# kangxiongbin/HyLight

Hardware: AMD Instinct MI355X
Metric: long-read all-vs-all overlaps/sec (higher is better)
Workload: dtype u8/int32

## Files before the change

### hylight_amd/csrc/ava.h

```cpp
#pragma once
#include <vector>

#include "common.h"
#include "paf_io.h"

namespace hlmi {

constexpr int CHAIN_PRED = 64;
constexpr int BLOCK_MIN = 32;
constexpr int BLOCK_MAX = 256;
constexpr int BAND_W = 64;
constexpr int BAND_PAD = 12;
constexpr int NARROW_W = 16;
constexpr int NARROW_PAD = 5;
constexpr int NARROW_DELTA = 5;
constexpr int EXT_MAX = 256;
constexpr int HALF_W = 32;
constexpr int HALF_DELTA = 7;
constexpr int ZDROP_STEP = 32;
constexpr int SHIFT_MAX = BAND_W - 2 * BAND_PAD - 1;
constexpr int MAX_MID_OCC = 1000000;
constexpr int NEG_INF = -(1 << 29);

inline int ext_rows(const hlmi_ava_opts &o) { return o.max_gap > EXT_MAX ? o.max_gap : EXT_MAX; }
inline int long_rows_cap(const hlmi_ava_opts &o) { return ext_rows(o) + BLOCK_MIN + SHIFT_MAX + BAND_W + 1; }

hlmi_ava_opts ava_opts_long();
hlmi_ava_opts ava_opts_short();

struct Mz {
    uint64_t x;
    uint64_t y;
};

struct DevReads {
    static constexpr size_t PAD = 64;
    size_t n = 0;
    uint64_t total = 0;
    DBuf<uint8_t> store;
    uint8_t *codes() const { return store.p + PAD; }
    void alloc_codes() {
        store.alloc(total + 2 * PAD);
        HIP_CHECK(hipMemsetAsync(store.p, 4, PAD, stream()));
        HIP_CHECK(hipMemsetAsync(store.p + PAD + total, 4, PAD, stream()));
    }
    DBuf<uint64_t> off;
    std::vector<uint64_t> h_off;
};
void upload_reads(const SeqSet &s, size_t lo, size_t hi, DevReads &out);
void upload_reads(const SeqSet &s, const std::vector<uint32_t> &ids, DevReads &out);
void subset_reads_device(const DevReads &all, const std::vector<uint32_t> &ids, DevReads &out);

struct DevSketch {
    size_t n = 0;
    DBuf<Mz> mz;
    DBuf<uint32_t> counts;
};
void sketch_device(const DevReads &r, int k, int w, int hpc, uint32_t rid_base, DevSketch &out);
int64_t sketch_device_into(const DevReads &r, int k, int w, int hpc, uint32_t rid_base, Mz *d_out, int64_t cap,
                           uint32_t *d_counts);

struct AvaInput {
    const DevReads *T = nullptr;
    const DevReads *Q = nullptr;
    const uint32_t *d_rank_t = nullptr;
    const uint32_t *d_rank_q = nullptr;
    uint64_t n_ranks = 0;
    const uint32_t *d_chunk_of_t = nullptr;
    uint32_t n_chunks = 1;
    const Mz *d_qmz = nullptr;
    std::vector<uint64_t> qmz_off;
    std::vector<uint32_t> t_query;
    uint64_t max_anchors = 0;
    uint64_t max_out_bytes = 0;
    int max_lanes = 0;
};
inline uint64_t ava_out_bytes(uint64_t rows, uint64_t ops) { return 4 * ops + 216 * rows; }

struct AvaRows {
    size_t n_rows = 0, n_ops = 0;
    DBuf<PafRec> recs;
    std::vector<DBuf<uint32_t>> ops_parts;
    std::vector<uint64_t> ops_part_len;
    const uint32_t *ops_base = nullptr;
    std::vector<uint64_t> chunk_row_start;
    uint64_t refused_anchors = 0;
    double refused_shrink = 1.0;
};
void ava_device(const AvaInput &in, const hlmi_ava_opts &o, AvaRows &out);

void ava_files(const char *target_fa, const char *query_fa, const hlmi_ava_opts &o, const char *out_paf);

void name_ranks(const std::vector<std::string> &a, const std::vector<std::string> &b, std::vector<uint32_t> &ra,
                std::vector<uint32_t> &rb, std::vector<std::string> &name_of_rank);

void format_ava_row(const PafRec &r, const uint32_t *ops, const std::string &qname, const std::string &tname,
                    std::string &out);

}
```

### hylight_amd/csrc/ava_align.hip

```cpp
#include <algorithm>
#include <memory>
#include <type_traits>

#include "ava_internal.h"
#include "dev_prims.h"
#include "wave_ops.h"

namespace hlmi {

namespace {
constexpr int WG = 256;
constexpr int WAVES = WG / 64;
constexpr int SEQ_T_MAX = EXT_MAX + BAND_W;
constexpr int NR_SHORT = 128;
constexpr int WIDE_SHORT = 128;
inline dim3 grid1(size_t n) { return dim3(cdiv(n ? n : 1, WG)); }

struct Task {
    uint32_t piece;
    uint16_t kind;
    uint16_t narrow;
    uint64_t qa, ta;
    int16_t m, n;
    int16_t dlo;
    int16_t trim;
};
constexpr uint16_t TASK_REV = 4;
constexpr uint16_t TASK_ONE = 8;
struct TaskOut {
    int32_t score;
    int32_t bi, bj;
    uint32_t runs_off, n_runs;
    uint32_t pad;
};
__device__ __forceinline__ uint32_t end_codes(uint32_t first_run, uint32_t last_run) { return (first_run & 15u) | (last_run & 15u) << 4; }

__global__ void piece_task_count_kernel(const Piece *pieces, size_t n, uint32_t *cnt) {
    size_t i = blockIdx.x * (size_t)blockDim.x + threadIdx.x;
    if (i < n) cnt[i] = pieces[i].n_fp + 1;
}

struct TaskRef { uint32_t pk, fp; };
struct PieceGeom {
    uint64_t qo, to;
    uint32_t ql, tl;
    uint32_t strand;
    uint32_t stub_cand;
};
struct TaskGeom {
    const TaskRef *ref;
    const PieceGeom *pg;
    const FixPt *fps;
};
__device__ __forceinline__ Task build_task(const PieceGeom &p, uint32_t piece, uint32_t kind, FixPt f0, FixPt f1, int ext_max) {
    const int ql = (int)p.ql, tl = (int)p.tl;
    const uint64_t qo = p.qo, to = p.to;
    const uint16_t rev = p.strand ? TASK_REV : 0;
    auto qaddr = [&](int pos) { return p.strand ? qo + (uint64_t)(ql - 1 - pos) : qo + (uint64_t)pos; };
    if (kind == 1) {
        const int qs = (int)f0.q, ts = (int)f0.t;
        const int m = qs < ext_max ? qs : ext_max, n2 = ts < m + BAND_W ? ts : m + BAND_W;
        return Task{piece, (uint16_t)(1u | rev), (uint16_t)(qs <= ext_max ? (qs + 1) << 1 : 0), qaddr(qs - 1),
                    to + (uint64_t)(ts - 1), (int16_t)m, (int16_t)n2, (int16_t)(-(BAND_W / 2 - 1)), 0};
    }
    if (kind == 2) {
        const int qe = (int)f0.q, te = (int)f0.t;
        const int m = ql - qe < ext_max ? ql - qe : ext_max, n2 = tl - te < m + BAND_W ? tl - te : m + BAND_W;
        return Task{piece, (uint16_t)(2u | rev), (uint16_t)(ql - qe <= ext_max ? (ql - qe + 1) << 1 : 0), qaddr(qe),
                    to + (uint64_t)te, (int16_t)m, (int16_t)n2, (int16_t)(-(BAND_W / 2 - 1)), 0};
    }
    const int q0 = (int)f0.q, t0 = (int)f0.t, m = (int)f1.q - q0, n2 = (int)f1.t - t0;
    const int delta = n2 - m, ad = delta < 0 ? -delta : delta;
    const bool lng = m > BLOCK_MAX || n2 > BLOCK_MAX;
    const bool narrow = !lng && ad <= NARROW_DELTA;
    const int lw = ad <= HALF_DELTA ? HALF_W : BAND_W;
    return Task{piece, rev, (uint16_t)(narrow ? 1 : 0), qaddr(q0), to + (uint64_t)t0, (int16_t)m, (int16_t)n2,
                (int16_t)((delta < 0 ? delta : 0) - (narrow ? NARROW_PAD : lng ? (lw - 1 - ad) / 2 : BAND_PAD)), 0};
}
__global__ __launch_bounds__(WG) void task_ref_kernel(const Piece *pieces, const uint32_t *task_off, size_t n, const uint32_t *qlen,
                                                       const uint32_t *tlen, const uint64_t *qoff, const uint64_t *toff,
                                                       const FixPt *fps, int stub_oh, int ext_max, TaskRef *task_ref, PieceGeom *pg) {
    const int lane = threadIdx.x & 63;
    const size_t wave = (blockIdx.x * (size_t)blockDim.x + threadIdx.x) >> 6;
    const size_t n_waves = ((size_t)gridDim.x * blockDim.x) >> 6;
    for (size_t i = wave; i < n; i += n_waves) {
        const Piece p = pieces[i];
        const uint32_t n_tasks = p.n_fp + 1;
        TaskRef *out = task_ref + task_off[i];
        for (uint32_t k = (uint32_t)lane; k < n_tasks; k += 64) {
            const uint32_t kind = k == 0 ? 1u : (k == p.n_fp ? 2u : 0u);
            out[k] = TaskRef{(uint32_t)i | kind << 30, p.fp_off + (k == 0 ? 0u : k - 1)};
        }
        if (lane == 0) {
            const uint32_t ql = qlen[p.q], tl = tlen[p.t];
            uint32_t cand = 0;
            if (stub_oh >= 0) {
                const FixPt a = fps[p.fp_off], b = fps[p.fp_off + p.n_fp - 1];
                const uint32_t dq = (uint32_t)(ext_max + stub_oh), dt = (uint32_t)(ext_max + BAND_W + stub_oh);
                cand = ((a.q > dq && a.t > dt) || (ql - b.q > dq && tl - b.t > dt)) ? 1u : 0u;
            }
            pg[i] = PieceGeom{qoff[p.q], toff[p.t], ql, tl, p.strand, cand};
        }
    }
}

__global__ __launch_bounds__(WG) void task_ref_lane_kernel(const Piece *pieces, const uint32_t *task_off, size_t n, const uint32_t *qlen,
                                                            const uint32_t *tlen, const uint64_t *qoff, const uint64_t *toff,
                                                            const FixPt *fps, int stub_oh, int ext_max, TaskRef *task_ref, PieceGeom *pg) {
    const size_t i = blockIdx.x * (size_t)blockDim.x + threadIdx.x;
    if (i >= n) return;
    const Piece p = pieces[i];
    const uint32_t n_tasks = p.n_fp + 1;
    TaskRef *out = task_ref + task_off[i];
    for (uint32_t k = 0; k < n_tasks; ++k) {
        const uint32_t kind = k == 0 ? 1u : (k == p.n_fp ? 2u : 0u);
        out[k] = TaskRef{(uint32_t)i | kind << 30, p.fp_off + (k == 0 ? 0u : k - 1)};
    }
    const uint32_t ql = qlen[p.q], tl = tlen[p.t];
    uint32_t cand = 0;
    if (stub_oh >= 0) {
        const FixPt a = fps[p.fp_off], b = fps[p.fp_off + p.n_fp - 1];
        const uint32_t dq = (uint32_t)(ext_max + stub_oh), dt = (uint32_t)(ext_max + BAND_W + stub_oh);
        cand = ((a.q > dq && a.t > dt) || (ql - b.q > dq && tl - b.t > dt)) ? 1u : 0u;
    }
    pg[i] = PieceGeom{qoff[p.q], toff[p.t], ql, tl, p.strand, cand};
}

struct AlignArgs {
    Task *tasks;
    TaskGeom geom;
    size_t n_tasks;
    const uint32_t *list;
    size_t n_list;
    const uint8_t *qcodes, *tcodes;
    long long q_total, t_total;
    int match, mismatch, go, ge, ambi;
    int go2, ge2;
    int end_bonus;
    int ext_max;
    int ext_all_long;
    int ungapped;
    int kmax;
    int kgap1;
    int kgap2;
    int one_ok;
    int kext_plain;
    int kext_bonus;
    int trim_ok;
    int kshift;
    TaskOut *out;
    uint32_t *runs;
    uint32_t cap_runs;
    uint32_t *counters;
    uint32_t run_buf_cap;
    uint8_t *cls_bare;
    uint8_t *defer_flag;
    const uint32_t *defer_list, *defer_count;
};

__device__ __forceinline__ uint32_t wave_excl_sum_u32(uint32_t v, int lane, uint32_t &total) {
    (void)lane;
    const uint32_t x = wave_prefix_sum_incl_dpp(v);
    total = (uint32_t)__builtin_amdgcn_readlane((int)x, 63);
    return x - v;
}

constexpr uint32_t RUN_CHUNK = 4096;
constexpr uint32_t RUN_CHUNK_SMALL = 256;
__device__ __forceinline__ uint32_t pool_take(const AlignArgs &a, uint32_t n, uint32_t &chunk_off, uint32_t &chunk_left,
                                              bool &ok, uint32_t chunk = RUN_CHUNK) {
    if (n > chunk_left) {
        const uint32_t want = n > chunk ? n : chunk;
        chunk_off = atomicAdd(&a.counters[0], want);
        chunk_left = want;
        if ((unsigned long long)chunk_off + want > a.cap_runs) { a.counters[1] = 1; chunk_left = 0; ok = false; return 0; }
    }
    const uint32_t off = chunk_off;
    chunk_off += n;
    chunk_left -= n;
    return off;
}

__device__ __forceinline__ uint32_t load_codes4(const uint8_t *base, long long idx, long long total) {
    if (idx >= 0 && idx + 4 <= total) {
        uint32_t v;
        __builtin_memcpy(&v, base + idx, 4);
        return v;
    }
    uint32_t v = 0;
    for (int k = 0; k < 4; ++k) v |= (uint32_t)(idx + k >= 0 && idx + k < total ? base[idx + k] : 4) << (8 * k);
    return v;
}
__device__ __forceinline__ uint32_t comp_codes4(uint32_t x) {
    const uint32_t n = x & 0x04040404u;
    return (x ^ 0x03030303u) & ~((n >> 1) | (n >> 2));
}
__device__ __forceinline__ uint32_t load_window4(const uint8_t *codes, long long total, long long a0, bool down, bool comp, int x) {
    uint32_t v = down ? __builtin_bswap32(load_codes4(codes, a0 - x - 3, total)) : load_codes4(codes, a0 + x, total);
    if (comp) v = comp_codes4(v);
    return v;
}

__device__ __forceinline__ uint32_t load_window4p(const uint8_t *codes, long long a0, bool down, bool comp, int x) {
    uint32_t v;
    __builtin_memcpy(&v, codes + (down ? a0 - x - 3 : a0 + x), 4);
    if (down) v = __builtin_bswap32(v);
    if (comp) v = comp_codes4(v);
    return v;
}


enum { ST_BASES = 0, ST_BASES_SQUARE, ST_BASES_NARROW, ST_BASES_WIDE, ST_FAST, ST_DP, ST_DP_ROWS, ST_NARROW_SMALL, ST_WIDE_ONE, ST_STUB_EXT, ST_EXT_CERT, ST_EXT_DP_ROW, ST_EXT_DP_K, ST_LONG, ST_BASES_LONG, N_ALIGN_STATS };
constexpr int NR_SMALL = 64;
constexpr uint8_t CLS_LONG = 5;
constexpr uint8_t CLS_LONG32 = 7;
constexpr uint8_t CLS_UNGAPPED = 6;

__device__ __forceinline__ uint64_t load_codes8(const uint8_t *base, long long idx, long long total) {
    if (idx >= 0 && idx + 8 <= total) {
        uint64_t v;
        __builtin_memcpy(&v, base + idx, 8);
        return v;
    }
    uint64_t v = 0;
    for (int k = 0; k < 8; ++k) v |= (uint64_t)(idx + k >= 0 && idx + k < total ? base[idx + k] : 4) << (8 * k);
    return v;
}
__device__ __forceinline__ uint64_t load_window8(const uint8_t *codes, long long total, long long a0, bool down, bool comp, int x) {
    uint64_t v = down ? __builtin_bswap64(load_codes8(codes, a0 - x - 7, total)) : load_codes8(codes, a0 + x, total);
    if (comp) {
        const uint64_t n = v & 0x0404040404040404ull;
        v = (v ^ 0x0303030303030303ull) & ~((n >> 1) | (n >> 2));
    }
    return v;
}

__device__ __forceinline__ uint64_t load_window8p(const uint8_t *codes, long long a0, bool down, bool comp, int x) {
    uint64_t v;
    __builtin_memcpy(&v, codes + (down ? a0 - x - 7 : a0 + x), 8);
    if (down) v = __builtin_bswap64(v);
    if (comp) {
        const uint64_t n = v & 0x0404040404040404ull;
        v = (v ^ 0x0303030303030303ull) & ~((n >> 1) | (n >> 2));
    }
    return v;
}

template <int PASS>
__global__ __launch_bounds__(WG) __attribute__((amdgpu_waves_per_eu(PASS == 1 ? 4 : 5))) void classify_kernel(AlignArgs a, uint8_t *cls, unsigned long long *stats) {
    __shared__ unsigned long long s_stat[WAVES][N_ALIGN_STATS];
    constexpr int CMP_PIECES = PASS == 1 ? 64 * (BLOCK_MAX / 8) : 1;
    __shared__ uint8_t s_mm[WAVES][CMP_PIECES], s_up[WAVES][CMP_PIECES], s_dn[WAVES][CMP_PIECES];
    __shared__ uint64_t s_qa[WAVES][PASS == 1 ? 64 : 1], s_ta[WAVES][PASS == 1 ? 64 : 1];
    __shared__ uint32_t s_geo[WAVES][PASS == 1 ? 64 : 1], s_amb[WAVES][2];
    const int lane = threadIdx.x & 63;
    const size_t tid = blockIdx.x * (size_t)blockDim.x + threadIdx.x;
    const size_t n_thr = (size_t)gridDim.x * blockDim.x;
    uint32_t chunk_off = 0, chunk_left = 0;
    uint32_t st[N_ALIGN_STATS] = {0, 0, 0, 0, 0, 0, 0, 0, 0, 0, 0, 0, 0, 0, 0};
    const size_t n_units = PASS == 1 ? a.n_tasks : (size_t)*a.defer_count;
    const size_t rounds = (n_units + n_thr - 1) / n_thr;
    TaskRef ref_n{0, 0};
    uint32_t ti_n = 0;
    if (PASS == 1) { if (tid < n_units) ref_n = a.geom.ref[tid]; }
    else if (tid < n_units) ti_n = a.defer_list[tid];
    for (size_t r = 0; r < rounds; ++r) {
        const size_t u = r * n_thr + tid;
        bool live = u < n_units;
        const size_t ti = PASS == 1 || !live ? u : (size_t)ti_n;
        TaskRef ref = ref_n;
        if (PASS == 2 && live) ref = a.geom.ref[ti];
        {
            const size_t un = u + n_thr;
            if (PASS == 1) { if (un < n_units) ref_n = a.geom.ref[un]; }
            else if (un < n_units) ti_n = a.defer_list[un];
        }
        Task tk{};
        bool held = false;
        bool bare = false;
        if (live) {
            const uint32_t pc = ref.pk & 0x3fffffffu, kind = ref.pk >> 30;
            const PieceGeom pg = a.geom.pg[pc];
            held = PASS == 1 && kind != 0 && pg.stub_cand != 0;
            bare = a.cls_bare != nullptr && pg.stub_cand != 0;
            const FixPt f0 = a.geom.fps[ref.fp];
            FixPt f1{0, 0};
            if (kind == 0) f1 = a.geom.fps[ref.fp + 1];
            tk = build_task(pg, pc, kind, f0, f1, a.ext_max);
        }
        const int m = tk.m, n = tk.n;
        uint8_t c = 2;
        bool try_fast = false;
        if (live) {
            if (m <= 0 || n <= 0 || held) c = 0;
            else if ((tk.kind & 3) == 0) {
                if (m > BLOCK_MAX || n > BLOCK_MAX)
                    c = (n > m ? n - m : m - n) <= HALF_DELTA ? CLS_LONG32 : CLS_LONG;
                else { c = tk.narrow ? (m <= NR_SHORT ? 1 : 3) : 2; try_fast = (m == n); }
            } else if ((m < n - tk.dlo ? m : n - tk.dlo) > EXT_MAX) { c = CLS_LONG32; tk.dlo = (int16_t)(-(HALF_W / 2 - 1)); }
            else if (a.ext_all_long) c = CLS_LONG;
            if (c == 2 && (m < n - tk.dlo ? m : n - tk.dlo) <= WIDE_SHORT) c = 4;
        }
        if (PASS == 1 && live) {
            const bool defer = c != 0 && a.kmax >= 0 && ((tk.kind & 3) != 0 || (m != n && c != CLS_LONG && c != CLS_LONG32));
            a.defer_flag[ti] = defer ? 1 : 0;
            if (defer) { live = false; try_fast = false; }
        }
        int k = 0, mpos[3] = {0, 0, 0}, last_x = -1;
        bool ambig = false, shift_ok = false;
        if constexpr (PASS == 1) {
            const int wv = threadIdx.x >> 6;
            uint8_t *own = s_mm[wv], *mm = s_mm[wv], *mup = s_up[wv], *mdn = s_dn[wv];
            const uint32_t nch = try_fast ? (uint32_t)(m + 7) >> 3 : 0u;
            const uint32_t incl = wave_prefix_sum_incl_dpp(nch), tot = (uint32_t)__builtin_amdgcn_readlane((int)incl, 63);
            const uint32_t st0 = incl - nch;
            for (uint32_t c = (uint32_t)lane; c < tot; c += 64) own[c] = 0;
            if (lane < 2) s_amb[wv][lane] = 0;
            s_qa[wv][lane] = tk.qa; s_ta[wv][lane] = tk.ta;
            s_geo[wv][lane] = st0 | (uint32_t)m << 16 | ((tk.kind & TASK_REV) ? 0x80000000u : 0u);
            __builtin_amdgcn_s_waitcnt(0xc07f);
            __builtin_amdgcn_wave_barrier();
            if (nch) own[st0] = (uint8_t)lane;
            __builtin_amdgcn_s_waitcnt(0xc07f);
            __builtin_amdgcn_wave_barrier();
            int carry = 0;
            constexpr int CU = 4;
            for (uint32_t c0 = 0; c0 < tot; c0 += 64 * CU) {
                int ow[CU], xs[CU], left[CU];
                bool rv[CU];
#pragma unroll
                for (int u = 0; u < CU; ++u) {
                    const uint32_t c = c0 + 64u * u + (uint32_t)lane;
                    int o = c < tot ? (int)own[c] : 0;
                    o = wave_prefix_max_incl_dpp(o);
                    o = o > carry ? o : carry;
                    carry = __builtin_amdgcn_readlane(o, 63);
                    const uint32_t geo = s_geo[wv][o];
                    ow[u] = o;
                    xs[u] = (int)(c - (geo & 0xffffu)) * 8;
                    left[u] = c < tot ? (int)(geo >> 16 & 0x7fffu) - xs[u] : 0;
                    rv[u] = (geo >> 31) != 0;
                }
                uint64_t q8[CU], t8[CU];
                uint32_t q_end = 0, t_end = 0;
#pragma unroll
                for (int u = 0; u < CU; ++u) {
                    q8[u] = t8[u] = 0;
                    if (left[u] > 0) {
                        q8[u] = load_window8p(a.qcodes, (long long)s_qa[wv][ow[u]], rv[u], rv[u], xs[u]);
                        t8[u] = load_window8p(a.tcodes, (long long)s_ta[wv][ow[u]], false, false, xs[u]);
                        if (u == CU - 1 && lane == 63 && a.kshift) {
                            q_end = (uint32_t)load_window8p(a.qcodes, (long long)s_qa[wv][ow[u]], rv[u], rv[u], xs[u] + 8) & 0xffu;
                            t_end = (uint32_t)load_window8p(a.tcodes, (long long)s_ta[wv][ow[u]], false, false, xs[u] + 8) & 0xffu;
                        }
                    }
                }
                int nq[CU], nt[CU];
                if (a.kshift) {
#pragma unroll
                    for (int u = 0; u < CU; ++u) {
                        const int q_after = u + 1 < CU ? __builtin_amdgcn_readlane((int)((uint32_t)q8[u + 1 < CU ? u + 1 : u] & 0xffu), 0) : (int)q_end;
                        const int t_after = u + 1 < CU ? __builtin_amdgcn_readlane((int)((uint32_t)t8[u + 1 < CU ? u + 1 : u] & 0xffu), 0) : (int)t_end;
                        nq[u] = wave_shl1((int)((uint32_t)q8[u] & 0xffu), q_after);
                        nt[u] = wave_shl1((int)((uint32_t)t8[u] & 0xffu), t_after);
                    }
                }
#pragma unroll
                for (int u = 0; u < CU; ++u) {
                    if (left[u] <= 0) continue;
                    const uint64_t keep = left[u] >= 8 ? ~0ull : (1ull << (8 * left[u])) - 1ull;
                    uint64_t d = (q8[u] ^ t8[u]) & keep;
                    if ((q8[u] | t8[u]) & keep & 0x0404040404040404ull) atomicOr(&s_amb[wv][ow[u] >> 5], 1u << (ow[u] & 31));
                    d = (d | d >> 1 | d >> 2) & 0x0101010101010101ull;
                    auto squeeze = [](uint64_t f) {
                        return (uint8_t)((((uint32_t)f * 0x10204080u) >> 28) | (((uint32_t)(f >> 32) * 0x10204080u) >> 28) << 4);
                    };
                    mm[c0 + 64u * u + (uint32_t)lane] = squeeze(d);
                    if (a.kshift) {
                        const uint64_t q9 = q8[u] >> 8 | (uint64_t)(uint32_t)nq[u] << 56, t9 = t8[u] >> 8 | (uint64_t)(uint32_t)nt[u] << 56;
                        uint64_t du = q9 ^ t8[u], dd = q8[u] ^ t9;
                        du = (du | du >> 1 | du >> 2) & 0x0101010101010101ull;
                        dd = (dd | dd >> 1 | dd >> 2) & 0x0101010101010101ull;
                        mup[c0 + 64u * u + (uint32_t)lane] = squeeze(du);
                        mdn[c0 + 64u * u + (uint32_t)lane] = squeeze(dd);
                    }
                }
            }
            __builtin_amdgcn_s_waitcnt(0xc07f);
            __builtin_amdgcn_wave_barrier();
            if (try_fast) {
                ambig = (s_amb[wv][lane >> 5] >> (lane & 31)) & 1u;
                for (uint32_t j = 0; j < nch && k <= a.kmax + a.kshift; ++j) {
                    uint32_t bits = mm[st0 + j];
                    while (bits) {
                        const int y = __ffs((int)bits) - 1;
                        bits &= bits - 1;
                        if (k < 3) mpos[k] = (int)(8 * j) + y;
                        ++k;
                    }
                }
            }
            if (try_fast && !ambig && a.kshift && k == a.kmax + 1) {
                const int p1 = mpos[0], pk = mpos[k - 1];
                uint32_t any_up = 0, any_dn = 0;
                for (int j = p1 >> 3; j <= (pk - 1) >> 3; ++j) {
                    uint32_t keepb = 0xffu;
                    if (j == p1 >> 3) keepb &= 0xffu << (p1 & 7);
                    if (j == (pk - 1) >> 3) keepb &= 0xffu >> (7 - ((pk - 1) & 7));
                    any_up |= mup[st0 + (uint32_t)j] & keepb;
                    any_dn |= mdn[st0 + (uint32_t)j] & keepb;
                }
                shift_ok = any_up != 0 && any_dn != 0;
            }
            if (try_fast && k > 0 && !ambig) {
                for (int j = (int)nch - 1; j >= 0; --j) {
                    const uint32_t bits = mm[st0 + (uint32_t)j];
                    if (bits) { last_x = 8 * j + 31 - __clz((int)bits); break; }
                }
            }
            __builtin_amdgcn_wave_barrier();
        }
        bool fast = try_fast && !ambig && k <= a.kmax;
        if (shift_ok) fast = true;
        uint32_t runs[7];
        uint32_t nr = 0;
        int fast_score = a.match * (m - k) - a.mismatch * k;
        uint32_t ext_flag = 0;
        int ext_take = -1;
        if (PASS == 2 && live && c != 0 && (tk.kind & 3) != 0 && a.kmax >= 0) {
            const bool rev = (tk.kind & TASK_REV) != 0, left = (tk.kind & 3) == 1;
            const int L = m < n ? m : n;
            const int end_row = (int)(tk.narrow >> 1) - 1;
            const bool bonus_row = a.end_bonus != 0 && end_row >= 0 && end_row <= n + (BAND_W / 2 - 1);
            bool same = !bonus_row || L == end_row;
            int allow = -1, k_ext = 0;
            bool amb_ext = false;
            if (a.go2 > 0 && a.ge > a.ge2 && a.end_bonus == 0 && a.one_ok) {
                int g = (a.go2 - a.go + (a.ge - a.ge2) - 1) / (a.ge - a.ge2);
                g = g < 1 ? 1 : g;
                allow = (a.go2 + a.ge2 * g - 1) / (a.match + a.mismatch);
            }
            const int k_want = bonus_row ? (L == end_row ? a.kext_bonus : 0) : a.kext_plain;
            int x1 = -1, x2 = -1;
            auto more = [&]() { return same || (!amb_ext && (k_ext <= allow || k_ext <= k_want)); };
            auto take8 = [&](int x, uint64_t q8, uint64_t t8) {
                const int rest = L - x;
                const uint64_t keep = rest >= 8 ? ~0ull : (1ull << (8 * rest)) - 1ull;
                uint64_t d = (q8 ^ t8) & keep;
                amb_ext |= ((q8 | t8) & keep & 0x0404040404040404ull) != 0;
                d = (d | d >> 1 | d >> 2) & 0x0101010101010101ull;
                if (d && x2 < 0) {
                    const int y1 = (__ffsll((long long)d) - 1) >> 3;
                    if (x1 < 0) { x1 = x + y1; const uint64_t d2 = d & (d - 1); if (d2) x2 = x + ((__ffsll((long long)d2) - 1) >> 3); }
                    else x2 = x + y1;
                }
                k_ext += __popcll(d);
                same = same && d == 0 && !amb_ext;
            };
            for (int x = 0; x < L && more(); x += 16) {
                const uint64_t q8 = load_window8p(a.qcodes, (long long)tk.qa, left != rev, rev, x);
                const uint64_t t8 = load_window8p(a.tcodes, (long long)tk.ta, left, false, x);
                uint64_t q8b = 0, t8b = 0;
                if (x + 8 < L) {
                    q8b = load_window8p(a.qcodes, (long long)tk.qa, left != rev, rev, x + 8);
                    t8b = load_window8p(a.tcodes, (long long)tk.ta, left, false, x + 8);
                }
                take8(x, q8, t8);
                if (x + 8 < L && more()) take8(x + 8, q8b, t8b);
            }
            if (!same && !amb_ext && k_ext <= allow) { tk.kind |= TASK_ONE; ++st[ST_WIDE_ONE]; }
            if (same) {
                runs[nr++] = (uint32_t)L << 4 | OP_EQ;
                fast_score = a.match * L;
                ext_flag = L == end_row ? 0x80000000u : 0u;
                fast = true;
                c = 0;
            } else if (!amb_ext && k_ext >= 1 && k_ext <= k_want) {
                int take = L;
                if (!bonus_row && a.match * x1 >= a.match * (L - 1) - a.mismatch) take = x1;
                const int subs = take == L ? k_ext : 0;
                int prev = 0;
                if (take > 0) {
                    if (subs >= 1) {
                        if (x1 > 0) runs[nr++] = (uint32_t)x1 << 4 | OP_EQ;
                        if (subs == 2 && x2 == x1 + 1) { runs[nr++] = 2u << 4 | OP_X; prev = x2 + 1; }
                        else {
                            runs[nr++] = 1u << 4 | OP_X; prev = x1 + 1;
                            if (subs == 2) {
                                runs[nr++] = (uint32_t)(x2 - prev) << 4 | OP_EQ;
                                runs[nr++] = 1u << 4 | OP_X; prev = x2 + 1;
                            }
                        }
                    }
                    if (take > prev) runs[nr++] = (uint32_t)(take - prev) << 4 | OP_EQ;
                }
                if (left) for (uint32_t i = 0; i < nr / 2; ++i) { const uint32_t v = runs[i]; runs[i] = runs[nr - 1 - i]; runs[nr - 1 - i] = v; }
                fast_score = a.match * (take - subs) - a.mismatch * subs;
                ext_flag = bonus_row && take == end_row ? 0x80000000u : 0u;
                ext_take = take;
                fast = true;
                c = 0;
                ++st[ST_EXT_CERT];
            } else if (bonus_row && L != end_row) ++st[ST_EXT_DP_ROW];
            else ++st[ST_EXT_DP_K];
        } else if (PASS == 2 && live && c != 0 && (tk.kind & 3) == 0 && m != n && a.kmax >= 0) {
            const bool rev = (tk.kind & TASK_REV) != 0;
            const int mn = m < n ? m : n, gap = n > m ? n - m : m - n;
            const bool del = n > m;
            const int want = a.kgap1 && gap == 1 ? (a.kgap2 ? 3 : 2) : 1;
            int found_a = 0, found_b = 0, a1 = mn, a2 = mn, a3 = mn, b1 = -1, b2 = -1, b3 = -1;
            bool amb = false;
            const int sq = m > n ? m - n : 0, st_ = n > m ? n - m : 0;
            for (int x = 0; x < mn && (found_a < want || found_b < want); x += 8) {
                const bool da = found_a < want, db = found_b < want;
                const int e0 = mn - 8 - x;
                uint64_t q8 = 0, t8 = 0, q8e = 0, t8e = 0;
                if (da) { q8 = load_window8p(a.qcodes, (long long)tk.qa, rev, rev, x); t8 = load_window8p(a.tcodes, (long long)tk.ta, false, false, x); }
                if (db) { q8e = load_window8p(a.qcodes, (long long)tk.qa, rev, rev, e0 + sq); t8e = load_window8p(a.tcodes, (long long)tk.ta, false, false, e0 + st_); }
                const int left = mn - x;
                if (da) {
                    const uint64_t keep = left >= 8 ? ~0ull : (1ull << (8 * left)) - 1ull;
                    amb |= ((q8 | t8) & keep & 0x0404040404040404ull) != 0;
                    uint64_t d = (q8 ^ t8) & keep;
                    d = (d | d >> 1 | d >> 2) & 0x0101010101010101ull;
                    while (d && found_a < want) {
                        const int y = (__ffsll((long long)d) - 1) >> 3;
                        d &= d - 1;
                        if (found_a == 0) a1 = x + y; else if (found_a == 1) a2 = x + y; else a3 = x + y;
                        ++found_a;
                    }
                }
                if (db) {
                    const uint64_t keep = left >= 8 ? ~0ull : ~0ull << (8 * (8 - left));
                    amb |= ((q8e | t8e) & keep & 0x0404040404040404ull) != 0;
                    uint64_t d = (q8e ^ t8e) & keep;
                    d = (d | d >> 1 | d >> 2) & 0x0101010101010101ull;
                    while (d && found_b < want) {
                        const int z = 7 - (__clzll((long long)d) >> 3);
                        d &= ~(0xffull << (8 * z));
                        if (found_b == 0) b1 = e0 + z; else if (found_b == 1) b2 = e0 + z; else b3 = e0 + z;
                        ++found_b;
                    }
                }
            }
            int p_star = -1, xpos = -1, xpos2 = -1;
            if (!amb) {
                if (b1 < a1) p_star = b1 + 1;
                else if (want >= 2 && b2 < a1) { p_star = b2 + 1; xpos = b1; }
                else if (want >= 2 && b1 < a2) { p_star = b1 + 1; xpos = a1; }
            }
            if (p_star < 0 && !amb && want == 3) {
                int ps = -1, x1 = -1, x2 = -1;
                const int mab = a1 < b2 ? a1 : b2, Mab = a1 > b2 ? a1 : b2, m2 = a2 < b1 ? a2 : b1, M2 = a2 > b1 ? a2 : b1;
                if (b2 >= 0 && b3 < mab) { ps = b3 + 1; x1 = b2; x2 = b1; }
                else if (a1 < mn && b1 >= 0 && Mab < m2) { ps = Mab + 1; x1 = a1; x2 = b1; }
                else if (a2 < mn && M2 < a3) { ps = M2 + 1; x1 = a1; x2 = a2; }
                if (ps >= 0 && a1 < b1) {
                    auto load_s = [&](int x) { return del ? load_window8p(a.qcodes, (long long)tk.qa, rev, rev, x) : load_window8p(a.tcodes, (long long)tk.ta, false, false, x); };
                    auto load_l = [&](int x) { return del ? load_window8p(a.tcodes, (long long)tk.ta, false, false, x) : load_window8p(a.qcodes, (long long)tk.qa, rev, rev, x); };
                    bool far_ne = false, near_ne = false, ambx = false;
                    for (int x = a1; x < b1 && !far_ne; x += 8) {
                        const uint64_t s8 = load_s(x), l8 = load_l(x + 2);
                        const int left = b1 - x;
                        const uint64_t keep = left >= 8 ? ~0ull : (1ull << (8 * left)) - 1ull;
                        ambx |= ((s8 | l8) & keep & 0x0404040404040404ull) != 0;
                        far_ne = ((s8 ^ l8) & keep) != 0;
                    }
                    for (int x = a1 + 1; x <= b1 && !near_ne; x += 8) {
                        const uint64_t s8 = load_s(x), l8 = load_l(x - 1);
                        const int left = b1 + 1 - x;
                        const uint64_t keep = left >= 8 ? ~0ull : (1ull << (8 * left)) - 1ull;
                        ambx |= ((s8 | l8) & keep & 0x0404040404040404ull) != 0;
                        near_ne = ((s8 ^ l8) & keep) != 0;
                    }
                    if (far_ne && near_ne && !ambx) { p_star = ps; xpos = x1; xpos2 = x2; }
                }
            }
            if (p_star < 0 && !amb && b1 >= 0) last_x = b1;
            if (p_star >= 0) {
                auto seg = [&](int from, int to) {
                    int prev = from;
                    for (int k = 0; k < 2; ++k) {
                        const int xp = k ? xpos2 : xpos;
                        if (xp < from || xp >= to) continue;
                        if (xp > prev) runs[nr++] = (uint32_t)(xp - prev) << 4 | OP_EQ;
                        if (nr && xp == prev && prev > from && (runs[nr - 1] & 15u) == OP_X) runs[nr - 1] += 1u << 4;
                        else runs[nr++] = 1u << 4 | OP_X;
                        prev = xp + 1;
                    }
                    if (to > prev) runs[nr++] = (uint32_t)(to - prev) << 4 | OP_EQ;
                };
                seg(0, p_star);
                runs[nr++] = (uint32_t)gap << 4 | (del ? OP_D : OP_I);
                seg(p_star, mn);
                const int subs = (xpos >= 0 ? 1 : 0) + (xpos2 >= 0 ? 1 : 0);
                int gap_cost = a.go + a.ge * gap;
                if (a.go2 && a.go2 + a.ge2 * gap < gap_cost) gap_cost = a.go2 + a.ge2 * gap;
                fast_score = a.match * (mn - subs) - a.mismatch * subs - gap_cost;
                fast = true;
                c = 0;
            }
        } else if (fast) {
            c = 0;
            int prev = 0, xs = -1, xe = -1;
            for (int i = 0; i < k; ++i) {
                const int x = mpos[i];
                if (x == xe) { xe = x + 1; continue; }
                if (xs >= 0) { runs[nr++] = (uint32_t)(xe - xs) << 4 | OP_X; prev = xe; }
                if (x > prev) runs[nr++] = (uint32_t)(x - prev) << 4 | OP_EQ;
                xs = x; xe = x + 1;
            }
            if (xs >= 0) { runs[nr++] = (uint32_t)(xe - xs) << 4 | OP_X; prev = xe; }
            if (m > prev) runs[nr++] = (uint32_t)(m - prev) << 4 | OP_EQ;
        }
        if (bare) nr = 0;
        uint32_t wave_total;
        const uint32_t mine = wave_excl_sum_u32(nr, lane, wave_total);
        uint32_t base = 0;
        bool ok = true;
        if (wave_total) {
            if (lane == 0) base = pool_take(a, wave_total, chunk_off, chunk_left, ok);
            base = (uint32_t)__shfl((int)base, 0, 64);
            ok = __shfl((int)ok, 0, 64) != 0;
        }
        if (fast) {
            if (ok) for (uint32_t q = 0; q < nr; ++q) a.runs[base + mine + q] = runs[q];
            const bool ext = (tk.kind & 3) != 0;
            const int L = ext_take >= 0 ? ext_take : (m < n ? m : n);
            a.out[ti] = TaskOut{fast_score, ext ? L : m, ext ? L : n, base + mine, ok ? nr : 0, (nr ? end_codes(runs[0], runs[nr - 1]) : 0u) | ext_flag};
        } else if (live && c == 0) {
            a.out[ti] = TaskOut{0, 0, 0, 0, 0, 0};
        }
        int m_dp = m;
        if (live && !fast && (c == 1 || c == 3) && a.kmax >= 0 && last_x >= 0 && a.trim_ok && !a.ungapped) {
            const int mn = m < n ? m : n;
            int T = mn - 1 - last_x;
            T = T < mn - 1 ? T : mn - 1;
            if (T > 0) {
                tk.m = (int16_t)(m - T); tk.n = (int16_t)(n - T); tk.trim = (int16_t)T;
                m_dp = m - T;
                c = m_dp <= NR_SHORT ? 1 : 3;
            }
        }
        if (live) {
            if (a.ungapped && c != 0) c = CLS_UNGAPPED;
            cls[ti] = bare ? 0 : c;
            if (a.cls_bare) a.cls_bare[ti] = bare ? c : 0;
            if (c != 0) a.tasks[ti] = tk;
            if (held) ++st[ST_STUB_EXT];
            else if (m > 0 && n > 0) {
                const uint32_t bases = (uint32_t)(m + n);
                st[ST_BASES] += bases;
                if ((tk.kind & 3) == 0 && m == n) st[ST_BASES_SQUARE] += bases;
                if (c == 0) ++st[ST_FAST];
                else {
                    ++st[ST_DP];
                    if (c == CLS_LONG || c == CLS_LONG32) { ++st[ST_LONG]; st[ST_BASES_LONG] += bases; st[ST_DP_ROWS] += (uint32_t)(m < n - tk.dlo ? m : n - tk.dlo); }
                    else if (c == 2 || c == 4) { st[ST_BASES_WIDE] += bases; st[ST_DP_ROWS] += (uint32_t)(m < n - tk.dlo ? m : n - tk.dlo); }
                    else { st[ST_BASES_NARROW] += bases; st[ST_DP_ROWS] += (uint32_t)m_dp; if (c == 1 && m_dp < NR_SMALL && !bare) ++st[ST_NARROW_SMALL]; }
                }
            }
        }
    }
#pragma unroll
    for (int k = 0; k < N_ALIGN_STATS; ++k) {
        unsigned long long v = st[k];
#pragma unroll
        for (int o = 32; o > 0; o >>= 1) v += __shfl_xor(v, o, 64);
        if (lane == 0) s_stat[threadIdx.x >> 6][k] = v;
    }
    __syncthreads();
    if (threadIdx.x < N_ALIGN_STATS) {
        unsigned long long v = 0;
        for (int w = 0; w < WAVES; ++w) v += s_stat[w][threadIdx.x];
        if (v) atomicAdd(&stats[threadIdx.x], v);
    }
}

__global__ void task_rows_key_kernel(const Task *tasks, const uint32_t *list, size_t n, uint32_t *key) {
    size_t i = blockIdx.x * (size_t)blockDim.x + threadIdx.x;
    if (i < n) key[i] = (uint32_t)tasks[list[i]].m >> 2;
}


__global__ void task_rows_desc_key_kernel(const Task *tasks, const uint32_t *list, size_t n, uint32_t *key) {
    size_t i = blockIdx.x * (size_t)blockDim.x + threadIdx.x;
    if (i >= n) return;
    const Task &t = tasks[list[i]];
    const int rows = (int)t.m < (int)t.n - (int)t.dlo ? (int)t.m : (int)t.n - (int)t.dlo;
    key[i] = 0xffffu - (uint32_t)(rows < 0 ? 0 : rows);
}

constexpr int DP_BIAS = 1 << 24;
constexpr int NT_PAD = 16;
constexpr int NT_EXTRA = NT_PAD + NARROW_DELTA + NARROW_W + 7;
enum { PL_DIAG = 0, PL_EGEF, PL_EEXT, PL_FEXT, PL_NE, N_PLANES };

__device__ __forceinline__ uint32_t shift_in(uint32_t acc, bool bit) {
#if defined(__HIP_DEVICE_COMPILE__)
    const unsigned long long m = __ballot(bit);
    unsigned long long co;
    asm("v_addc_co_u32 %0, %1, %2, %2, %3" : "=v"(acc), "=s"(co) : "v"(acc), "s"(m));
#endif
    return acc;
}

struct NarrowWalk {
    const uint32_t *pl;
    int chunks;
    int lb;
    int m, n, dlo;
    int wmask;
    bool keep_order;
    int trim;
    __device__ __forceinline__ uint32_t word(int plane, int c, int lane) const { return pl[(plane * chunks + c) * 64 + lane]; }
};
struct WalkScore {
    int match, mismatch, go, ge;
    int total;
};
__device__ uint32_t narrow_walk(const NarrowWalk &w, uint32_t *out, uint32_t total, uint32_t *buf = nullptr, uint32_t cap = 0,
                                WalkScore *ws = nullptr, uint32_t *ends = nullptr) {
    int i = w.m, j = w.n, state = 0;
    uint32_t cur_op = OP_EQ, cur_len = (uint32_t)w.trim, n_runs = 0, e_first = 0, e_last = 0;
    auto put = [&]() {
        if (!n_runs) e_first = cur_op;
        e_last = cur_op;
        if (out) out[w.keep_order ? n_runs : total - 1 - n_runs] = cur_len << 4 | cur_op;
        else if (n_runs < cap) buf[n_runs] = cur_len << 4 | cur_op;
        ++n_runs;
        if (ws) ws->total += cur_op == OP_EQ ? ws->match * (int)cur_len
                           : (cur_op == OP_X ? -ws->mismatch * (int)cur_len : -(ws->go + ws->ge * (int)cur_len));
    };
    for (int it = 0; (i > 0 || j > 0) && it < 4 * (EXT_MAX + SEQ_T_MAX); ++it) {
        uint32_t op, len;
        if (i == 0) {
            op = OP_D; len = (uint32_t)j; j = 0;
        } else {
            const int d = w.lb + ((j - i - w.dlo) & w.wmask);
            const int c = (i - 1) >> 5, sh = 31 - ((i - 1) & 31);
            const uint32_t dg = w.word(PL_DIAG, c, d) >> sh;
            const uint32_t ne = w.word(PL_NE, c, d) >> sh;
            const uint32_t eg = w.word(PL_EGEF, c, d) >> sh;
            const uint32_t ee = w.word(PL_EEXT, c, (d - 1) & 63) >> sh;
            const int i2 = i > 1 ? i - 2 : 0;
            const uint32_t fe = w.word(PL_FEXT, i2 >> 5, (d + 1) & 63) >> (31 - (i2 & 31));
            const int st = state != 0 ? state : ((dg & 1u) ? 0 : ((eg & 1u) ? 1 : 2));
            if (st == 0) {
                const uint32_t inv = ~dg;
                const int r = inv ? __ffs((int)inv) - 1 : 32;
                const bool isx = (ne & 1u) != 0;
                const uint32_t flip = isx ? ~ne : ne;
                int l = flip ? __ffs((int)flip) - 1 : 32;
                l = l < r ? l : r;
                op = isx ? OP_X : OP_EQ; len = (uint32_t)l;
                i -= l; j -= l;
                state = 0;
            } else if (st == 1) {
                op = OP_D; len = 1;
                state = (ee & 1u) ? 1 : 0;
                --j;
            } else {
                op = OP_I; len = 1;
                state = (i > 1 && (fe & 1u)) ? 2 : 0;
                --i;
            }
        }
        if (op == cur_op) cur_len += len;
        else { if (cur_len) put(); cur_op = op; cur_len = len; }
    }
    if (cur_len) put();
    if (ends) *ends = w.keep_order ? end_codes(e_first, e_last) : end_codes(e_last, e_first);
    return n_runs;
}
constexpr int RUN_BUF_NARROW = 48, RUN_BUF_WIDE = 128;

template <bool AMBI, int NR_CHUNKS>
__device__ __forceinline__ void narrow_rows(const AlignArgs &a, int rows, int m, int dlo, int l, const uint8_t *sq,
                                            const uint8_t *st, uint32_t (*pl)[NR_CHUNKS][64], int lane, int &Hend) {
    const int go = a.go, ge = a.ge, goe = go + ge, gel = ge * l, goel = go + ge * l;
    const int j0 = dlo + l;
    int H = j0 == 0 ? DP_BIAS : (j0 > 0 ? DP_BIAS - (go + ge * j0) : 0);
    int G = H - goe;
    uint32_t a0 = 0, a1 = 0, a2 = 0, a3 = 0, a4 = 0;
    const uint8_t *tp = st + NT_PAD + dlo + l - 1;
    int v_match = a.match, v_mis = -a.mismatch;
    asm volatile("" : "+v"(v_match), "+v"(v_mis));
    auto row = [&](int i, int qa, int t2) {
        const bool ne = qa != t2;
        int s = ne ? v_mis : v_match;
        if (AMBI) s = (qa | t2) > 3 ? -a.ambi : s;
        const int mm = H + s;
        const int f = row_shl1_z(G);
        const int ht = mm > f ? mm : f;
        const int e = row_shr1(row_prefix_max_incl_dpp(ht + gel), 0) - goel;
        const int h = ht > e ? ht : e;
        const int fo = h - goe, fe = f - ge;
        a0 = shift_in(a0, mm == h);
        a1 = shift_in(a1, e >= f);
        a2 = shift_in(a2, e + go > h);
        a3 = shift_in(a3, fe > fo);
        a4 = shift_in(a4, ne);
        G = fo > fe ? fo : fe;
        H = h;
        if (i == m) Hend = h;
    };
    int qa = sq[0], t2 = tp[1];
    int i = 1;
    for (; i < rows; i += 2) {
        const int qb = sq[i], tb = tp[i + 1], qc = sq[i + 1], tc = tp[i + 2];
        row(i, qa, t2);
        row(i + 1, qb, tb);
        qa = qc; t2 = tc;
        if (((i + 1) & 31) == 0) {
            const int c = ((i + 1) >> 5) - 1;
            pl[PL_DIAG][c][lane] = a0; pl[PL_EGEF][c][lane] = a1; pl[PL_EEXT][c][lane] = a2; pl[PL_FEXT][c][lane] = a3;
            pl[PL_NE][c][lane] = a4;
        }
    }
    if (i == rows) row(i, qa, t2);
    if (rows & 31) {
        const int c = rows >> 5, up = 32 - (rows & 31);
        pl[PL_DIAG][c][lane] = a0 << up; pl[PL_EGEF][c][lane] = a1 << up; pl[PL_EEXT][c][lane] = a2 << up;
        pl[PL_FEXT][c][lane] = a3 << up; pl[PL_NE][c][lane] = a4 << up;
    }
}

template <int NR_MAX>
__global__ __launch_bounds__(WG) void align_narrow_kernel(AlignArgs a) {
    constexpr int NR_CHUNKS = NR_MAX / 32, NQ_STEPS = NR_MAX / 64, NT_STEPS = NR_MAX / 64 + 1;
    __shared__ uint32_t s_pl[WAVES][N_PLANES][NR_CHUNKS][64];
    __shared__ __attribute__((aligned(4))) uint8_t s_q[WAVES * 4][NR_MAX + 4];
    __shared__ __attribute__((aligned(4))) uint8_t s_t[WAVES * 4][NR_MAX + NT_EXTRA];
    __shared__ uint32_t s_runs[WAVES * 4][RUN_BUF_NARROW];
    const int lane = threadIdx.x & 63, g = lane >> 4, l = lane & 15, wv = threadIdx.x >> 6;
    const size_t wave = (blockIdx.x * (size_t)blockDim.x + threadIdx.x) >> 6;
    const size_t n_waves = ((size_t)gridDim.x * blockDim.x) >> 6;
    uint32_t (*pl)[NR_CHUNKS][64] = s_pl[wv];
    uint8_t *sq = s_q[wv * 4 + g], *st = s_t[wv * 4 + g];
    uint32_t chunk_off = 0, chunk_left = 0;
    const size_t n_quads = (a.n_list + 3) / 4;
    for (size_t qd = wave; qd < n_quads; qd += n_waves) {
        const size_t li = qd * 4 + g;
        const bool live = li < a.n_list;
        size_t ti = 0;
        Task tk{};
        if (live) { ti = a.list[li]; tk = a.tasks[ti]; }
        const int m = tk.m, n = tk.n, dlo = tk.dlo;
        bool ambig = false;
        if (live) {
            const bool rev = (tk.kind & TASK_REV) != 0;
            uint32_t vq[NQ_STEPS], vt[NT_STEPS];
#pragma unroll
            for (int r = 0; r < NQ_STEPS; ++r) {
                const int x = 4 * (l + 16 * r);
                vq[r] = 0;
                if (x < m) vq[r] = load_window4p(a.qcodes, (long long)tk.qa, rev, rev, x);
            }
#pragma unroll
            for (int r = 0; r < NT_STEPS; ++r) {
                const int x = 4 * (l + 16 * r);
                vt[r] = 0;
                if (x < n) vt[r] = load_window4p(a.tcodes, (long long)tk.ta, false, false, x);
            }
#pragma unroll
            for (int r = 0; r < NQ_STEPS; ++r) {
                const int x = 4 * (l + 16 * r);
                if (x < m) { *(uint32_t *)(sq + x) = vq[r]; ambig |= (vq[r] & 0x04040404u) != 0; }
            }
#pragma unroll
            for (int r = 0; r < NT_STEPS; ++r) {
                const int x = 4 * (l + 16 * r);
                if (x < n) { *(uint32_t *)(st + NT_PAD + x) = vt[r]; ambig |= (vt[r] & 0x04040404u) != 0; }
            }
        }
        __builtin_amdgcn_s_waitcnt(0);
        __builtin_amdgcn_wave_barrier();
// ... 1232 lines not shown

template <bool WRITE>
__global__ __launch_bounds__(WG) void assemble_lane_kernel(AsmArgs a, uint32_t *n_ops, uint8_t *valid, const uint64_t *ops_off,
                                                            uint32_t *ops, PafRec *recs, uint64_t *ord_hi, uint64_t *ord_lo) {
    const size_t idx = blockIdx.x * (size_t)blockDim.x + threadIdx.x;
    if (idx >= a.n_pieces) return;
    const size_t i = !WRITE && a.plist ? (size_t)a.plist[idx] : idx;
    if (WRITE && !valid[i]) return;
    const Piece p = a.pieces[i];
    const FixPt *fp = a.fps + p.fp_off;
    const TaskOut *to = a.tout + a.task_off[i];
    const uint32_t n_tasks = p.n_fp + 1;
    const bool bare = a.bare && a.pg[i].stub_cand != 0;
    uint32_t *w = WRITE ? ops + ops_off[i] : nullptr;
    long long score = 0;
    unsigned long long nmatch = 0, blen = 0;
    uint32_t slots = 0;
    uint32_t pend = 0;
    uint32_t carry_code = 99;
    int li = 0, lj = 0, ri = 0, rj = 0;
    for (uint32_t t = 0; t < n_tasks; ++t) {
        const TaskOut r = to[t];
        bool keep = true;
        if (t == 0 || t == n_tasks - 1)
            keep = !(r.score + ((r.pad & 0x80000000u) ? a.end_bonus : 0) <= 0 || (r.n_runs == 0 && !bare));
        if (!keep) continue;
        if (t == 0) { li = r.bi; lj = r.bj; }
        else if (t == n_tasks - 1) { ri = r.bi; rj = r.bj; }
        score += r.score;
        const uint32_t nr = bare ? 0u : r.n_runs;
        if (!nr) continue;
        const uint32_t first = r.pad & 15u, last = (r.pad >> 4) & 15u;
        const bool mrg = first == carry_code;
        carry_code = last;
        if (!WRITE) {
            slots += nr - (mrg ? 1u : 0u);
            continue;
        }
        for (uint32_t x = 0; x < nr; ++x) {
            const uint32_t run = a.runs[r.runs_off + x];
            blen += run >> 4;
            if ((run & 15u) == OP_EQ) nmatch += run >> 4;
            if (x == 0 && mrg) pend += (run >> 4) << 4;
            else {
                if (pend) w[slots++] = pend;
                pend = run;
            }
        }
    }
    if (!WRITE) {
        const bool ok = (slots > 0 || bare) && score >= a.min_dp_score;
        valid[i] = ok ? 1 : 0;
        n_ops[i] = ok ? slots : 0;
        if (a.late) a.late[i] = a.pg[i].stub_cand && !((slots > 0 || bare) && score >= a.stub_score) ? 1 : 0;
        return;
    }
    if (pend) w[slots++] = pend;
    const int qs = (int)fp[0].q - li, ts = (int)fp[0].t - lj;
    const int qe = (int)fp[p.n_fp - 1].q + ri, te = (int)fp[p.n_fp - 1].t + rj;
    const uint32_t ql = a.qlen[p.q];
    PafRec r{};
    r.qid = a.rank_q[p.q]; r.tid = a.rank_t[p.t];
    r.qlen = ql; r.tlen = a.tlen[p.t];
    r.qs = p.strand ? ql - (uint32_t)qe : (uint32_t)qs;
    r.qe = p.strand ? ql - (uint32_t)qs : (uint32_t)qe;
    r.ts = (uint32_t)ts; r.te = (uint32_t)te;
    r.nmatch = (uint32_t)nmatch; r.blen = (uint32_t)blen;
    r.flags = p.strand ? PF_REV : 0;
    r.chunk = a.chunk_of_t[p.t];
    r.cig_off = ops_off[i]; r.cig_n = slots; r.tie = 0;
    recs[i] = r;
    ord_hi[i] = (uint64_t)r.chunk << 32 | p.q;
    ord_lo[i] = (uint64_t)p.t << 43 | (uint64_t)p.strand << 42 | (uint64_t)(p.chain & 0x3fffffu) << 20 | (p.piece & 0xfffffu);
}

__global__ void late_tasks_kernel(const uint32_t *plist, size_t n, const Piece *pieces, const uint32_t *task_off, uint32_t *tasks,
                                  uint32_t *count) {
    size_t j = blockIdx.x * (size_t)blockDim.x + threadIdx.x;
    if (j == 0) *count = (uint32_t)(2 * n);
    if (j >= n) return;
    const uint32_t i = plist[j];
    tasks[2 * j] = task_off[i];
    tasks[2 * j + 1] = task_off[i] + pieces[i].n_fp;
}

__global__ __launch_bounds__(WG) void class_bases_kernel(const uint8_t *cls, const uint8_t *cls_bare, const Task *tasks, size_t n,
                                                          unsigned long long *out) {
    __shared__ unsigned long long s_sum[14];
    if (threadIdx.x < 14) s_sum[threadIdx.x] = 0;
    __syncthreads();
    for (size_t i = blockIdx.x * (size_t)blockDim.x + threadIdx.x; i < n; i += (size_t)gridDim.x * blockDim.x) {
        const int c = cls[i], cb = cls_bare ? cls_bare[i] : 0;
        if (!c && !cb) continue;
        const Task &t = tasks[i];
        int slot;
        if (c) slot = c == 1 ? ((int)t.m < NR_SMALL ? 0 : 1) : c == 3 ? 2 : c == 2 ? 3 : c == 4 ? 4 : c == CLS_LONG ? 5 : c == CLS_LONG32 ? 12 : 11;
        else slot = cb == 1 ? 6 : cb == 3 ? 7 : cb == 2 ? 8 : cb == 4 ? 9 : cb == CLS_LONG ? 10 : cb == CLS_LONG32 ? 13 : 11;
        atomicAdd(&s_sum[slot], (unsigned long long)((int)t.m + (int)t.n));
    }
    __syncthreads();
    if (threadIdx.x < 14 && s_sum[threadIdx.x]) atomicAdd(&out[threadIdx.x], s_sum[threadIdx.x]);
}

__global__ __launch_bounds__(WG) void list_ext_kernel(const Task *tasks, const uint32_t *list, size_t n, unsigned long long *out) {
    unsigned long long c = 0, r = 0;
    for (size_t i = blockIdx.x * (size_t)blockDim.x + threadIdx.x; i < n; i += (size_t)gridDim.x * blockDim.x) {
        const Task &t = tasks[list[i]];
        if (t.kind & 3) { ++c; r += (unsigned long long)(int)t.m; }
    }
#pragma unroll
    for (int o = 32; o > 0; o >>= 1) { c += __shfl_xor(c, o, 64); r += __shfl_xor(r, o, 64); }
    if ((threadIdx.x & 63) == 0 && c) { atomicAdd(out, c); atomicAdd(out + 1, r); }
}

__global__ void class_flag_kernel(const uint8_t *cls, size_t n, uint8_t v, uint8_t *flag) {
    size_t i = blockIdx.x * (size_t)blockDim.x + threadIdx.x;
    if (i < n) flag[i] = cls[i] == v ? 1 : 0;
}

__global__ void compact_rows_kernel(const uint32_t *idx, size_t n, const PafRec *recs, const uint64_t *hi,
                                    const uint64_t *lo, PafRec *orecs, uint64_t *ohi, uint64_t *olo) {
    size_t i = blockIdx.x * (size_t)blockDim.x + threadIdx.x;
    if (i >= n) return;
    orecs[i] = recs[idx[i]];
    ohi[i] = hi[idx[i]];
    olo[i] = lo[idx[i]];
}

__global__ __launch_bounds__(WG) void piece_long_flag_kernel(const Piece *pieces, size_t n, const FixPt *fps, const uint32_t *qlen,
                                                              const uint32_t *tlen, int ext_max, uint8_t *flag) {
    const int lane = threadIdx.x & 63;
    const size_t wave = (blockIdx.x * (size_t)blockDim.x + threadIdx.x) >> 6;
    const size_t n_waves = ((size_t)gridDim.x * blockDim.x) >> 6;
    for (size_t i = wave; i < n; i += n_waves) {
        const Piece p = pieces[i];
        const FixPt *fp = fps + p.fp_off;
        bool lng = false;
        if (lane == 0) {
            const FixPt a = fp[0], b = fp[p.n_fp - 1];
            const int ql = (int)qlen[p.q], tl = (int)tlen[p.t];
            auto rows = [&](int aq, int at) {
                const int m = aq < ext_max ? aq : ext_max, nn = at < m + BAND_W ? at : m + BAND_W;
                return m < nn + (BAND_W / 2 - 1) ? m : nn + (BAND_W / 2 - 1);
            };
            lng = rows((int)a.q, (int)a.t) > EXT_MAX || rows(ql - (int)b.q, tl - (int)b.t) > EXT_MAX;
        }
        for (uint32_t k = (uint32_t)lane; k + 1 < p.n_fp && !__any(lng); k += 64) {
            const FixPt f0 = fp[k], f1 = fp[k + 1];
            lng = lng || (int)(f1.q - f0.q) > BLOCK_MAX || (int)(f1.t - f0.t) > BLOCK_MAX;
        }
        const bool any = __any(lng);
        if (lane == 0) flag[i] = any ? 1 : 0;
    }
}
__global__ __launch_bounds__(WG) void piece_long_flag_lane_kernel(const Piece *pieces, size_t n, const FixPt *fps, const uint32_t *qlen,
                                                                   const uint32_t *tlen, int ext_max, uint8_t *flag) {
    const size_t i = blockIdx.x * (size_t)blockDim.x + threadIdx.x;
    if (i >= n) return;
    const Piece p = pieces[i];
    const FixPt *fp = fps + p.fp_off;
    FixPt f0 = fp[0];
    const FixPt b = fp[p.n_fp - 1];
    const int ql = (int)qlen[p.q], tl = (int)tlen[p.t];
    auto rows = [&](int aq, int at) {
        const int m = aq < ext_max ? aq : ext_max, nn = at < m + BAND_W ? at : m + BAND_W;
        return m < nn + (BAND_W / 2 - 1) ? m : nn + (BAND_W / 2 - 1);
    };
    bool lng = rows((int)f0.q, (int)f0.t) > EXT_MAX || rows(ql - (int)b.q, tl - (int)b.t) > EXT_MAX;
    for (uint32_t k = 1; k < p.n_fp && !lng; ++k) {
        const FixPt f1 = fp[k];
        lng = (int)(f1.q - f0.q) > BLOCK_MAX || (int)(f1.t - f0.t) > BLOCK_MAX;
        f0 = f1;
    }
    flag[i] = lng ? 1 : 0;
}
__global__ void gather_pieces_kernel(const Piece *src, const uint32_t *idx, size_t n, Piece *dst, uint32_t *n_fp) {
    size_t i = blockIdx.x * (size_t)blockDim.x + threadIdx.x;
    if (i >= n) return;
    const Piece p = src[idx[i]];
    dst[i] = p;
    if (n_fp) n_fp[i] = p.n_fp;
}
__global__ __launch_bounds__(WG) void move_fixed_points_kernel(Piece *pieces, size_t n, const uint32_t *off, uint32_t fp_base, const FixPt *src,
                                                                FixPt *dst) {
    const int lane = threadIdx.x & 63;
    const size_t wave = (blockIdx.x * (size_t)blockDim.x + threadIdx.x) >> 6;
    const size_t n_waves = ((size_t)gridDim.x * blockDim.x) >> 6;
    for (size_t i = wave; i < n; i += n_waves) {
        const Piece p = pieces[i];
        const uint32_t to = off[i];
        for (uint32_t k = (uint32_t)lane; k < p.n_fp; k += 64) dst[to + k] = src[p.fp_off + k];
        if (lane == 0) pieces[i].fp_off = fp_base + to;
    }
}
}

struct PieceSpan { struct { const Piece *p; } pieces; size_t n_pieces, n_fp; struct { const FixPt *p; } fps; };
static void align_span(const AvaInput &in, const hlmi_ava_opts &o, const uint32_t *d_qlen, const uint32_t *d_tlen,
                       const PieceSpan &ch, AlignOut &out) {
    out = AlignOut();
    const size_t P = ch.n_pieces;
    if (!P) return;
    DBuf<uint32_t> tcnt(P), toff(P);
    hipLaunchKernelGGL(piece_task_count_kernel, grid1(P), dim3(WG), 0, stream(), ch.pieces.p, P, tcnt.p);
    exclusive_scan_u32(tcnt.p, toff.p, P);
    const size_t NT = ch.n_fp + P;
    DBuf<Task> tasks(NT);
    if (P >= (1u << 30)) fail(HLMI_EINVAL, "more than 2^30 alignment pieces in one batch");
    DBuf<TaskRef> task_ref(NT);
    DBuf<PieceGeom> pgeom(P);
    if (NT <= 17 * P)
        hipLaunchKernelGGL(task_ref_lane_kernel, grid1(P), dim3(WG), 0, stream(), ch.pieces.p, toff.p, P, d_qlen, d_tlen, in.Q->off.p, in.T->off.p,
                           ch.fps.p, o.stub_oh, ext_rows(o), task_ref.p, pgeom.p);
    else
    hipLaunchKernelGGL(task_ref_kernel, dim3((unsigned)std::min<size_t>(cdiv(P, (size_t)WAVES), 256 * 32)), dim3(WG), 0, stream(),
                       ch.pieces.p, toff.p, P, d_qlen, d_tlen, in.Q->off.p, in.T->off.p, ch.fps.p, o.stub_oh, ext_rows(o), task_ref.p, pgeom.p);
    HIP_CHECK(hipGetLastError());
    DBuf<TaskOut> tout(NT);
    DBuf<uint32_t> counters(2);
    DBuf<unsigned long long> astats(N_ALIGN_STATS);
    constexpr size_t MAX_BLOCKS = 256 * 16;
    const size_t open_chunks = MAX_BLOCKS * (4 * WAVES * RUN_CHUNK + 2 * 4 * WAVES * RUN_CHUNK_SMALL) +
                               (size_t)3 * 256 * 32 * 8 * PK_WAVES * RUN_CHUNK_SMALL;
    size_t run_share = std::max<size_t>(NT * 12, 1 << 16);
    DBuf<uint32_t> runs;
    AsmArgs as{};
    as.pieces = ch.pieces.p; as.fps = ch.fps.p; as.task_off = toff.p; as.tout = tout.p; as.n_pieces = P;
    as.min_dp_score = o.min_dp_score; as.end_bonus = o.end_bonus;
    as.qlen = d_qlen; as.tlen = d_tlen; as.rank_q = in.d_rank_q; as.rank_t = in.d_rank_t; as.chunk_of_t = in.d_chunk_of_t;
    as.pg = pgeom.p; as.stub_score = o.min_dp_score + std::max(0, o.end_bonus);
    as.stage_cap = (uint32_t)ASM_STAGE;
    if (const char *e = hook("HLMI_ASM_STAGE_CAP")) as.stage_cap = (uint32_t)std::min(ASM_STAGE, std::max(0, atoi(e)));
    DBuf<uint32_t> nops(P);
    DBuf<uint8_t> valid(P), late(o.stub_oh >= 0 ? P : 0);
    DBuf<uint32_t> late_idx(o.stub_oh >= 0 ? P : 0);
    size_t n_late = 0;
    const unsigned nba = (unsigned)std::min<size_t>(cdiv(P, (size_t)WAVES), 256 * 32);
    const bool small_pieces = NT <= 17 * P && !hook("HLMI_ASM_WAVE");
    const int worst = std::max(std::max(o.match, o.mismatch), std::max(o.ambi, o.gap_open + o.gap_ext));
    const bool packed = worst > 0 && (long long)worst * (BLOCK_MAX + NARROW_W + 2) <= 4000 && o.match >= 0 && o.mismatch >= 0 &&
                        o.ambi >= 0 && o.gap_open >= 0 && o.gap_ext >= 0 && !hook("HLMI_NARROW_UNPACKED");
    const bool bare = o.stub_oh >= 0 && packed && !hook("HLMI_STUB_FULL_ROWS");
    as.bare = bare ? 1 : 0;
    if (long_rows_cap(o) > 32000) fail(HLMI_EINVAL, "max_gap %d: alignment tasks are limited to 32 000 rows", o.max_gap);
    bool ext_all_long = false;
    if (o.zdrop > 0) {
        const int D = std::max(std::max(o.mismatch, o.ambi), o.gap_open + o.gap_ext);
        const int rows_down = D > 0 ? (o.zdrop + D - 1) / D : EXT_MAX;
        ext_all_long = (long long)o.match * (EXT_MAX - rows_down) + std::max(o.end_bonus, 0) > o.zdrop;
    }
    const uint32_t long_chunks_cap = (uint32_t)(long_rows_cap(o) + 31) / 32, long_runs_cap = (uint32_t)(2 * long_rows_cap(o) + 64);
    constexpr unsigned LONG_BLOCKS_MAX = 256 * 8;
    struct LongLaunch { DBuf<uint32_t> list, planes, runs, ctl; };
    std::vector<std::unique_ptr<LongLaunch>> long_launches;
    struct LongReady { AlignArgs al; LongArgs la; unsigned nb; bool half, tb; const char *timer; };
    std::vector<LongReady> long_ready;
    hipEvent_t long_done = nullptr;
    bool long_pending = false, long_on_side = false;
    struct SideGuard {
        ~SideGuard() { if (hipStream_t s = side_stream_if_created()) (void)hipStreamSynchronize(s); }
    } side_guard;
    auto join_long = [&]() {
        if (!long_pending) return;
        if (long_on_side) {
            if (!long_done) HIP_CHECK(hipEventCreateWithFlags(&long_done, hipEventDisableTiming));
            HIP_CHECK(hipEventRecord(long_done, side_stream()));
            HIP_CHECK(hipStreamWaitEvent(stream(), long_done, 0));
            long_on_side = false;
        }
        long_pending = false;
    };
    DBuf<uint8_t> long_flag;
    DBuf<uint32_t> long_list, long_n(1);
    size_t n_long_tb = 0, n_long_bare = 0;
    double long_rows_run = 0;
    static const char *const LB_NAMES[] = {"align_narrow_small", "align_narrow", "align_narrow_long", "align_wide", "align_wide_short",
                                           "align_long", "align_score_narrow", "align_score_narrow_long", "align_score_wide",
                                           "align_score_wide_short", "align_score_long", "align_ungapped", "align_long32",
                                           "align_score_long32"};
    constexpr int N_LB = 14;
    DBuf<unsigned long long> lb_bases(N_LB + 2);
    std::vector<double> lb_n(N_LB, 0.0);
    lb_bases.zero();
    auto note_list = [&](const char *timer, const Task *tk, const uint32_t *lst, size_t n) {
        if (!n) return;
        int slot = 0;
        while (slot < N_LB && strcmp(LB_NAMES[slot], timer) != 0) ++slot;
        if (slot == N_LB) return;
        lb_n[slot] += (double)n;
        (void)tk; (void)lst;
    };
    for (int attempt = 0;; ++attempt) {
        const size_t cap_runs = run_share + open_chunks;
        if (cap_runs >= (1ull << 32)) fail(HLMI_ENOMEM, "CIGAR run pool exceeds 4G entries");
        runs.alloc(cap_runs);
        counters.zero();
        lb_bases.zero();
        std::fill(lb_n.begin(), lb_n.end(), 0.0);
        AlignArgs aa{};
        aa.tasks = tasks.p; aa.n_tasks = NT;
        aa.geom = TaskGeom{task_ref.p, pgeom.p, ch.fps.p};
        aa.qcodes = in.Q->codes(); aa.tcodes = in.T->codes();
        aa.q_total = (long long)in.Q->total; aa.t_total = (long long)in.T->total;
        aa.end_bonus = o.end_bonus;
        aa.ext_max = ext_rows(o);
        aa.ext_all_long = ext_all_long ? 1 : 0;
        aa.ungapped = o.bandwidth == 0 ? 1 : 0;
        aa.match = o.match; aa.mismatch = o.mismatch; aa.go = o.gap_open; aa.ge = o.gap_ext; aa.ambi = o.ambi;
        aa.go2 = o.gap_open2 > 0 ? o.gap_open2 : 0; aa.ge2 = o.gap_open2 > 0 ? o.gap_ext2 : 0;
        if (aa.go2 && aa.go2 + aa.ge2 * (NARROW_W - 1) < aa.go + aa.ge * (NARROW_W - 1))
            fail(HLMI_EINVAL, "two-piece gap cost: the second piece must not be the cheaper one below %d bases", NARROW_W);
        {
            const int den = o.match + o.mismatch, num = o.match + 2 * (o.gap_open + o.gap_ext);
            aa.kmax = den > 0 && num > 0 ? std::min(3, (num - 1) / den) : 0;
            if (o.match <= 0 || o.gap_open < 0 || o.gap_ext <= 0) aa.kmax = -1;
            const int k = aa.kmax + 1, U = den, T = num;
            aa.kgap1 = aa.kmax >= 0 && U < o.gap_open + 2 * o.gap_ext + o.match && !hook("HLMI_NO_GAP1_CERT") ? 1 : 0;
            {
                auto c = [&](int L) { int v = o.gap_open + o.gap_ext * L; if (o.gap_open2 > 0) v = std::min(v, o.gap_open2 + o.gap_ext2 * L); return v; };
                aa.kgap2 = aa.kgap1 && U < o.match + c(2) && 2 * U < o.match + 2 * c(1) && 2 * U < 2 * o.match + c(2) + c(3) - c(1) &&
                           c(2) == o.gap_open + 2 * o.gap_ext && c(1) == o.gap_open + o.gap_ext && !hook("HLMI_NO_GAP2_CERT") ? 1 : 0;
            }
            aa.kshift = aa.kmax >= 0 && k <= 3 && k * U > T && k * U < T + o.match + std::min(2 * o.gap_ext, o.gap_open + o.gap_ext) &&
                        !hook("HLMI_NO_SHIFT_CERT") ? 1 : 0;
        }
        aa.trim_ok = hook("HLMI_NO_SUFFIX_TRIM") ? 0 : 1;
        aa.one_ok = hook("HLMI_NO_ONE_PIECE_CERT") ? 0 : 1;
        {
            const int U = o.match + o.mismatch;
            int G = o.gap_open + o.gap_ext;
            if (aa.go2 > 0) G = std::min(G, aa.go2 + aa.ge2);
            const bool sane = aa.kmax >= 0 && o.match > 0 && o.mismatch >= 0 && !hook("HLMI_NO_EXT_CERT");
            aa.kext_plain = sane && G >= U && U < 2 * G + o.match ? 1 : 0;
            aa.kext_bonus = 0;
            for (int k = 1; k <= 2; ++k)
                if (sane && o.end_bonus > 0 && k * U < G && k * U < o.end_bonus + o.match && k * U < 2 * G + o.match) aa.kext_bonus = k;
        }
        aa.out = tout.p; aa.runs = runs.p; aa.cap_runs = (uint32_t)cap_runs; aa.counters = counters.p;
        as.runs = runs.p;
        aa.run_buf_cap = 0xffffffffu;
        if (const char *e = hook("HLMI_RUN_BUF_CAP")) aa.run_buf_cap = (uint32_t)std::max(0, atoi(e));
        DBuf<uint8_t> cls(NT), f1(NT), cls_bare(bare ? NT : 0);
        DBuf<uint32_t> list1(NT), list2(NT), list3(NT), list4(NT);
        DBuf<uint32_t> list_n(4);
        aa.cls_bare = bare ? cls_bare.p : nullptr;
        auto class_list = [&](const uint8_t *cls_arr, uint8_t v) -> size_t {
            if (long_flag.n < NT) { long_flag.alloc(NT); long_list.alloc(NT); }
            hipLaunchKernelGGL(class_flag_kernel, grid1(NT), dim3(WG), 0, stream(), cls_arr, NT, v, long_flag.p);
            select_flagged_indices_async(long_flag.p, long_list.p, NT, long_n.p);
            return (size_t)long_n.download(1)[0];
        };
        auto run_ungapped = [&](const uint8_t *cls_arr, bool tb) -> size_t {
            if (!aa.ungapped) return 0;
            const size_t nl = class_list(cls_arr, CLS_UNGAPPED);
            if (!nl) return 0;
            aa.list = long_list.p; aa.n_list = nl;
            note_list("align_ungapped", tasks.p, long_list.p, nl);
            KTimer kt("align_ungapped");
            const unsigned nb = (unsigned)std::min<size_t>(cdiv(nl, (size_t)WG), MAX_BLOCKS);
            if (tb) hipLaunchKernelGGL(align_ungapped_kernel<true>, dim3(nb), dim3(WG), 0, stream(), aa, o.zdrop);
            else hipLaunchKernelGGL(align_ungapped_kernel<false>, dim3(nb), dim3(WG), 0, stream(), aa, o.zdrop);
            HIP_CHECK(hipGetLastError());
            return nl;
        };
        auto run_long_class = [&](const uint8_t *cls_arr, bool tb, uint8_t cv) -> size_t {
            const bool half = cv == CLS_LONG32;
            const char *timer = half ? (tb ? "align_long32" : "align_score_long32") : (tb ? "align_long" : "align_score_long");
            const size_t nl = class_list(cls_arr, cv);
            if (!nl) return 0;
            note_list(timer, tasks.p, long_list.p, nl);
            hipLaunchKernelGGL(list_ext_kernel, dim3((unsigned)std::min<size_t>(cdiv(nl, (size_t)WG), 1024)), dim3(WG), 0, stream(), tasks.p,
                               long_list.p, nl, lb_bases.p + N_LB);
            long_launches.emplace_back(new LongLaunch());
            LongLaunch &L = *long_launches.back();
            {
                DBuf<uint32_t> key(nl);
                hipLaunchKernelGGL(task_rows_desc_key_kernel, grid1(nl), dim3(WG), 0, stream(), tasks.p, long_list.p, nl, key.p);
                L.list.alloc(nl);
                HIP_CHECK(hipMemcpyAsync(L.list.p, long_list.p, nl * 4, hipMemcpyDeviceToDevice, stream()));
                sort_pairs_u32_u32(key, L.list, nl, 0, 16);
            }
            const size_t units = half ? (nl + 1) / 2 : nl;
            const unsigned nb = (unsigned)std::min<size_t>((units + WAVES - 1) / WAVES, LONG_BLOCKS_MAX);
            const size_t n_waves = (size_t)nb * WAVES;
            LongArgs la{};
            if (tb) {
                L.planes.alloc(n_waves * (size_t)N_WPLANES * long_chunks_cap * 64);
                L.runs.alloc(n_waves * (size_t)long_runs_cap * (half ? 2 : 1));
                la.planes = L.planes.p; la.run_scratch = L.runs.p;
            }
            la.chunks_cap = long_chunks_cap; la.runs_cap = long_runs_cap; la.zdrop = o.zdrop;
            L.ctl.alloc(4);
            L.ctl.zero();
            la.next = L.ctl.p; la.too_long = L.ctl.p + 1; la.rows_run = (unsigned long long *)(L.ctl.p + 2);
            AlignArgs al = aa;
            al.list = L.list.p; al.n_list = nl;
            long_ready.push_back(LongReady{al, la, nb, half, tb, timer});
            return nl;
        };
        auto launch_long_ready = [&]() {
            if (long_ready.empty()) return;
            sync();
            const bool on_side = hook("HLMI_LONG_SIDE_STREAM") != nullptr;
            hipStream_t ls = on_side ? side_stream() : stream();
            long_on_side = long_on_side || on_side;
            for (const LongReady &r : long_ready) {
                KTimer kt(r.timer, ls);
                const bool two = aa.go2 > 0;
                auto go = [&](auto kern) { hipLaunchKernelGGL(kern, dim3(r.nb), dim3(WG), 0, ls, r.al, r.la); };
                if (r.half) {
                    if (r.tb) go(align_long32_kernel<false, true>); else go(align_long32_kernel<false, false>);
                } else {
                    if (r.tb) { if (two) go(align_long_kernel<true, true>); else go(align_long_kernel<false, true>); }
                    else { if (two) go(align_long_kernel<true, false>); else go(align_long_kernel<false, false>); }
                }
            }
            HIP_CHECK(hipGetLastError());
            long_ready.clear();
            long_pending = true;
        };
        auto run_long = [&](const uint8_t *cls_arr, bool tb) -> size_t {
            if (aa.ungapped) return run_ungapped(cls_arr, tb);
            const size_t n32 = run_long_class(cls_arr, tb, CLS_LONG32);
            return n32 + run_long_class(cls_arr, tb, CLS_LONG);
        };
        auto check_long = [&]() {
            for (auto &L : long_launches) {
                if (!L->ctl.n) continue;
                const std::vector<uint32_t> c = L->ctl.download(4);
                if (c[1]) fail(HLMI_EINVAL, "an alignment task exceeds the scratch area of align_long_kernel");
                long_rows_run += (double)((unsigned long long)c[3] << 32 | c[2]);
                L->ctl.release(); L->planes.release(); L->runs.release(); L->list.release();
            }
        };
        size_t n_bare_tasks = 0;
        auto run_bare_long = [&]() {
            if (!bare) return;
            const size_t nl = run_long(cls_bare.p, false);
            n_bare_tasks += nl; n_long_bare += nl;
        };
        auto run_bare = [&](bool with_long) {
            if (!bare) return;
            if (with_long) { run_bare_long(); launch_long_ready(); }
            select_classes4_async(cls_bare.p, NT, list1.p, list2.p, list3.p, list4.p, list_n.p);
            const std::vector<uint32_t> hb = list_n.download(4);
            n_bare_tasks += (size_t)hb[0] + hb[1] + hb[2] + hb[3];
            for (int which = 0; which < 2; ++which) {
                DBuf<uint32_t> &lst = which ? list3 : list1;
                const size_t nl = which ? hb[2] : hb[0];
                if (nl < 8) continue;
                DBuf<uint32_t> key(nl);
                hipLaunchKernelGGL(task_rows_key_kernel, grid1(nl), dim3(WG), 0, stream(), tasks.p, lst.p, nl, key.p);
                sort_pairs_u32_u32(key, lst, nl, 0, 7);
            }
            auto pk_grid = [](size_t n) { return dim3((unsigned)std::max<size_t>(1, std::min<size_t>(((n + 7) / 8 + PK_WAVES - 1) / PK_WAVES, 256 * 32))); };
            auto w_grid = [](size_t n) { return dim3((unsigned)std::max<size_t>(1, std::min<size_t>((n + WAVES - 1) / WAVES, 256 * 16))); };
            if (hb[0]) {
                note_list("align_score_narrow", tasks.p, list1.p, hb[0]);
                KTimer kt("align_score_narrow");
                aa.list = list1.p; aa.n_list = hb[0];
                hipLaunchKernelGGL((align_narrow_pk_kernel<NR_SHORT, false>), pk_grid(hb[0]), dim3(64 * PK_WAVES), 0, stream(), aa);
            }
            if (hb[2]) {
                note_list("align_score_narrow_long", tasks.p, list3.p, hb[2]);
                KTimer kt("align_score_narrow_long");
                aa.list = list3.p; aa.n_list = hb[2];
                hipLaunchKernelGGL((align_narrow_pk_kernel<BLOCK_MAX, false>), pk_grid(hb[2]), dim3(64 * PK_WAVES), 0, stream(), aa);
            }
            if (hb[1]) {
                note_list("align_score_wide", tasks.p, list2.p, hb[1]);
                KTimer kt("align_score_wide");
                aa.list = list2.p; aa.n_list = hb[1];
                hipLaunchKernelGGL((align_kernel<EXT_MAX, false>), w_grid(hb[1]), dim3(WG), 0, stream(), aa);
            }
            if (hb[3]) {
                note_list("align_score_wide_short", tasks.p, list4.p, hb[3]);
                KTimer kt("align_score_wide_short");
                aa.list = list4.p; aa.n_list = hb[3];
                hipLaunchKernelGGL((align_kernel<WIDE_SHORT, false>), w_grid(hb[3]), dim3(WG), 0, stream(), aa);
            }
        };
        {
            KTimer kt("align_classify");
            const unsigned nbc = (unsigned)std::min<size_t>(cdiv(NT, (size_t)WG), MAX_BLOCKS);
            astats.zero();
            aa.defer_flag = f1.p;
            aa.defer_list = list1.p; aa.defer_count = list_n.p;
            hipLaunchKernelGGL(classify_kernel<1>, dim3(nbc ? nbc : 1), dim3(WG), 0, stream(), aa, cls.p, astats.p);
            select_flagged_indices_async(f1.p, list1.p, NT, list_n.p);
            const unsigned nb2 = std::max(1u, nbc / 4);
            hipLaunchKernelGGL(classify_kernel<2>, dim3(nb2), dim3(WG), 0, stream(), aa, cls.p, astats.p);
        }
        HIP_CHECK(hipGetLastError());
        hipLaunchKernelGGL(class_bases_kernel, dim3((unsigned)std::min<size_t>(cdiv(NT, (size_t)WG), 2048)), dim3(WG), 0, stream(), cls.p,
                           bare ? cls_bare.p : nullptr, tasks.p, NT, lb_bases.p);
        select_classes4_async(cls.p, NT, list1.p, list2.p, list3.p, list4.p, list_n.p);
        const std::vector<uint32_t> hn = list_n.download(4);
        const size_t n1 = hn[0], n2 = hn[1], n3 = hn[2], n4 = hn[3];
        for (int which = 0; which < 2; ++which) {
            DBuf<uint32_t> &lst = which ? list3 : list1;
            const size_t nl = which ? n3 : n1;
            if (nl < 8) continue;
            DBuf<uint32_t> key(nl);
            hipLaunchKernelGGL(task_rows_key_kernel, grid1(nl), dim3(WG), 0, stream(), tasks.p, lst.p, nl, key.p);
            sort_pairs_u32_u32(key, lst, nl, 0, 7);
        }
        unsigned long long long_seen = astats.download(N_ALIGN_STATS)[ST_LONG];
        if (long_seen || aa.ungapped) {
            run_bare_long();
            n_long_tb += run_long(cls.p, true);
            launch_long_ready();
        }
        if (n1 && packed) {
            size_t n_small = 0;
            if (n1 >= 8) n_small = std::min<size_t>(n1, (size_t)astats.download(N_ALIGN_STATS)[ST_NARROW_SMALL]);
            if (n_small) {
                note_list("align_narrow_small", tasks.p, list1.p, n_small);
                KTimer kt("align_narrow_small");
                aa.list = list1.p; aa.n_list = n_small;
                const unsigned nb = (unsigned)std::min<size_t>(((n_small + 7) / 8 + PK_WAVES - 1) / PK_WAVES, 256 * 32);
                hipLaunchKernelGGL(align_narrow_pk_kernel<NR_SMALL>, dim3(nb ? nb : 1), dim3(64 * PK_WAVES), 0, stream(), aa);
            }
            if (n1 > n_small) {
                note_list("align_narrow", tasks.p, list1.p + n_small, n1 - n_small);
                KTimer kt("align_narrow");
                aa.list = list1.p + n_small; aa.n_list = n1 - n_small;
                const unsigned nb = (unsigned)std::min<size_t>(((aa.n_list + 7) / 8 + PK_WAVES - 1) / PK_WAVES, 256 * 32);
                hipLaunchKernelGGL(align_narrow_pk_kernel<NR_SHORT>, dim3(nb ? nb : 1), dim3(64 * PK_WAVES), 0, stream(), aa);
            }
        } else if (n1) {
            note_list("align_narrow", tasks.p, list1.p, n1);
            KTimer kt("align_narrow");
            aa.list = list1.p; aa.n_list = n1;
            const unsigned nb = (unsigned)std::min<size_t>(((n1 + 3) / 4 + WAVES - 1) / WAVES, 256 * 16);
            hipLaunchKernelGGL(align_narrow_kernel<NR_SHORT>, dim3(nb ? nb : 1), dim3(WG), 0, stream(), aa);
        }
        if (n3 && packed && !hook("HLMI_NARROW_LONG_UNPACKED")) {
            note_list("align_narrow_long", tasks.p, list3.p, n3);
            KTimer kt("align_narrow_long");
            aa.list = list3.p; aa.n_list = n3;
            const unsigned nb = (unsigned)std::min<size_t>(((n3 + 7) / 8 + PK_WAVES - 1) / PK_WAVES, 256 * 32);
            hipLaunchKernelGGL(align_narrow_pk_kernel<BLOCK_MAX>, dim3(nb ? nb : 1), dim3(64 * PK_WAVES), 0, stream(), aa);
        } else if (n3) {
            note_list("align_narrow_long", tasks.p, list3.p, n3);
            KTimer kt("align_narrow_long");
            aa.list = list3.p; aa.n_list = n3;
            const unsigned nb = (unsigned)std::min<size_t>(((n3 + 3) / 4 + WAVES - 1) / WAVES, 256 * 16);
            hipLaunchKernelGGL(align_narrow_kernel<BLOCK_MAX>, dim3(nb ? nb : 1), dim3(WG), 0, stream(), aa);
        }
        auto run_wide = [&](size_t n_long, size_t n_short) {
            if (n_long) {
                note_list("align_wide", tasks.p, list2.p, n_long);
                KTimer kt("align_wide");
                aa.list = list2.p; aa.n_list = n_long;
                const unsigned nb = (unsigned)std::min<size_t>((n_long + WAVES - 1) / WAVES, 256 * 16);
                hipLaunchKernelGGL(align_kernel<EXT_MAX>, dim3(nb ? nb : 1), dim3(WG), 0, stream(), aa);
            }
            if (n_short) {
                note_list("align_wide_short", tasks.p, list4.p, n_short);
                KTimer kt("align_wide_short");
                aa.list = list4.p; aa.n_list = n_short;
                const unsigned nb = (unsigned)std::min<size_t>((n_short + WAVES - 1) / WAVES, 256 * 16);
                hipLaunchKernelGGL(align_kernel<WIDE_SHORT>, dim3(nb ? nb : 1), dim3(WG), 0, stream(), aa);
            }
        };
        run_wide(n2, n4);
        run_bare(false);
        size_t n_wide_late = 0;
        if (o.stub_oh >= 0) {
            as.plist = nullptr; as.n_pieces = P; as.late = late.p;
            join_long();
            {
                KTimer kt("assemble_count");
                if (small_pieces) hipLaunchKernelGGL(assemble_lane_kernel<false>, grid1(as.n_pieces), dim3(WG), 0, stream(), as, nops.p, valid.p,
                                                     nullptr, nullptr, nullptr, nullptr, nullptr);
                else
                hipLaunchKernelGGL(assemble_kernel<false>, dim3(nba), dim3(WG), 0, stream(), as, nops.p, valid.p, nullptr, nullptr,
                                   nullptr, nullptr, nullptr);
            }
            as.late = nullptr;
            n_late = select_flagged_indices(late.p, late_idx.p, P);
            if (n_late) {
                hipLaunchKernelGGL(late_tasks_kernel, grid1(n_late), dim3(WG), 0, stream(), late_idx.p, n_late, ch.pieces.p, toff.p,
                                   list1.p, list_n.p);
                HIP_CHECK(hipMemsetAsync(cls.p, 0, NT, stream()));
                if (bare) HIP_CHECK(hipMemsetAsync(cls_bare.p, 0, NT, stream()));
                {
                    KTimer kt("align_classify");
                    aa.defer_list = list1.p; aa.defer_count = list_n.p;
                    const unsigned nb2 = (unsigned)std::min<size_t>(cdiv(2 * n_late, (size_t)WG), MAX_BLOCKS);
                    hipLaunchKernelGGL(classify_kernel<2>, dim3(nb2 ? nb2 : 1), dim3(WG), 0, stream(), aa, cls.p, astats.p);
                }
                hipLaunchKernelGGL(class_bases_kernel, dim3((unsigned)std::min<size_t>(cdiv(NT, (size_t)WG), 2048)), dim3(WG), 0, stream(), cls.p,
                                   bare ? cls_bare.p : nullptr, tasks.p, NT, lb_bases.p);
                if (bare) {
                    const size_t before = n_bare_tasks;
                    const bool more_long = astats.download(N_ALIGN_STATS)[ST_LONG] > long_seen || aa.ungapped;
                    run_bare(more_long);
                    n_wide_late = n_bare_tasks - before;
                } else {
                    select_classes4_async(cls.p, NT, list1.p, list2.p, list3.p, list4.p, list_n.p);
                    const std::vector<uint32_t> hl = list_n.download(4);
                    run_wide(hl[1], hl[3]);
                    const bool more_long = astats.download(N_ALIGN_STATS)[ST_LONG] > long_seen || aa.ungapped;
                    const size_t nl = more_long ? run_long(cls.p, true) : 0;
                    launch_long_ready();
                    n_long_tb += nl;
                    n_wide_late = (size_t)hl[1] + hl[3] + nl;
                }
                as.plist = late_idx.p; as.n_pieces = n_late;
                const unsigned nbl = (unsigned)std::min<size_t>(cdiv(n_late, (size_t)WAVES), 256 * 32);
                join_long();
                {
                    KTimer kt("assemble_count");
                    if (small_pieces) hipLaunchKernelGGL(assemble_lane_kernel<false>, grid1(as.n_pieces), dim3(WG), 0, stream(), as, nops.p, valid.p,
                                                         nullptr, nullptr, nullptr, nullptr, nullptr);
                    else
                    hipLaunchKernelGGL(assemble_kernel<false>, dim3(nbl), dim3(WG), 0, stream(), as, nops.p, valid.p, nullptr, nullptr,
                                       nullptr, nullptr, nullptr);
                }
                as.plist = nullptr; as.n_pieces = P;
            }
        }
        if (attempt == 0) {
            stat_add("align_tasks_narrow", (double)(n1 + n3)); stat_add("align_tasks_wide", (double)(n2 + n4 + (bare ? 0 : n_wide_late)));
            stat_add("align_tasks_score_only", (double)n_bare_tasks);
            stat_add("align_tasks_long", (double)n_long_tb); stat_add("align_tasks_long_score_only", (double)n_long_bare);
        }
        HIP_CHECK(hipGetLastError());
        join_long();
        std::vector<uint32_t> hc = counters.download(2);
        check_long();
        if (!hc[1]) break;
        if (attempt >= 3) fail(HLMI_ENOMEM, "CIGAR run pool overflow");
        run_share *= 4;
    }
    stat_add("align_tasks", (double)NT);
    {
        std::vector<unsigned long long> h = astats.download(N_ALIGN_STATS);
        stat_add("align_tasks_fast", (double)h[ST_FAST]);
        stat_add("align_tasks_dp", (double)h[ST_DP]);
        stat_add("align_dp_rows", (double)h[ST_DP_ROWS]);
        stat_add("align_dp_bases", (double)h[ST_BASES]);
        stat_add("align_bases_classify", (double)h[ST_BASES_SQUARE]);
        stat_add("align_bases_narrow", (double)h[ST_BASES_NARROW]);
        stat_add("align_bases_wide", (double)h[ST_BASES_WIDE]);
        stat_add("align_bases_long", (double)h[ST_BASES_LONG]);
        const std::vector<unsigned long long> lb = lb_bases.download(N_LB + 2);
        stat_add("align_long_rows_run", long_rows_run);
        stat_add("align_long_ext", (double)lb[N_LB]);
        stat_add("align_long_ext_rows", (double)lb[N_LB + 1]);
        for (int k = 0; k < N_LB; ++k)
            if (lb_n[k] > 0) {
                stat_add(std::string("align_n.") + LB_NAMES[k], lb_n[k]);
                stat_add(std::string("align_bases.") + LB_NAMES[k], (double)lb[k]);
            }
        stat_add("align_tasks_wide_one_piece", (double)h[ST_WIDE_ONE]);
        stat_add("align_ext_certified", (double)h[ST_EXT_CERT]);
        stat_add("align_ext_dp_bonus_row_elsewhere", (double)h[ST_EXT_DP_ROW]);
        stat_add("align_ext_dp_substitutions", (double)h[ST_EXT_DP_K]);
        stat_add("align_ext_held", (double)h[ST_STUB_EXT]);
        stat_add("align_ext_late", (double)(2 * n_late));
    }
    if (o.stub_oh < 0) {
        KTimer kt("assemble_count");
        if (small_pieces) hipLaunchKernelGGL(assemble_lane_kernel<false>, grid1(as.n_pieces), dim3(WG), 0, stream(), as, nops.p, valid.p,
                                             nullptr, nullptr, nullptr, nullptr, nullptr);
        else
        hipLaunchKernelGGL(assemble_kernel<false>, dim3(nba), dim3(WG), 0, stream(), as, nops.p, valid.p, nullptr, nullptr,
                           nullptr, nullptr, nullptr);
    }
    HIP_CHECK(hipGetLastError());
    DBuf<uint64_t> ooff(P);
    exclusive_scan_u32_to_u64(nops.p, ooff.p, P);
    const size_t n_ops = (size_t)(download_one(ooff.p + (P - 1)) + download_one(nops.p + (P - 1)));
    DBuf<uint32_t> vidx(P);
    const size_t R = select_flagged_indices(valid.p, vidx.p, P);
    if (!R) return;
    out.ops.alloc(n_ops ? n_ops : 1);
    DBuf<PafRec> recs(P);
    DBuf<uint64_t> hi(P), lo(P);
    {
        KTimer kt("assemble_write");
        if (small_pieces) hipLaunchKernelGGL(assemble_lane_kernel<true>, grid1(as.n_pieces), dim3(WG), 0, stream(), as, nullptr, valid.p, ooff.p,
                                             out.ops.p, recs.p, hi.p, lo.p);
        else
        hipLaunchKernelGGL(assemble_kernel<true>, dim3(nba), dim3(WG), 0, stream(), as, nullptr, valid.p, ooff.p, out.ops.p,
                           recs.p, hi.p, lo.p);
    }
    HIP_CHECK(hipGetLastError());
    out.recs.alloc(R);
    out.ord_hi.alloc(R);
    out.ord_lo.alloc(R);
    hipLaunchKernelGGL(compact_rows_kernel, grid1(R), dim3(WG), 0, stream(), vidx.p, R, recs.p, hi.p, lo.p, out.recs.p,
                       out.ord_hi.p, out.ord_lo.p);
    HIP_CHECK(hipGetLastError());
    sync();
    out.n_rows = R;
    out.n_ops = n_ops;
}

}

namespace hlmi {
void align_pieces(const AvaInput &in, const hlmi_ava_opts &o, const uint32_t *d_qlen, const uint32_t *d_tlen,
                  const ChainOut &ch_in, std::vector<AlignOut> &outs, DeferredPieces *defer) {
    if (!ch_in.n_pieces) return;
    ChainOut kept;
    const ChainOut *chp = &ch_in;
    if (defer && o.bandwidth != 0) {
        const size_t P0 = ch_in.n_pieces;
        DBuf<uint8_t> flag(P0), nflag(P0);
        if (ch_in.n_fp <= 16 * P0)
            hipLaunchKernelGGL(piece_long_flag_lane_kernel, grid1(P0), dim3(WG), 0, stream(), ch_in.pieces.p, P0, ch_in.fps.p, d_qlen, d_tlen,
                               ext_rows(o), flag.p);
        else
        hipLaunchKernelGGL(piece_long_flag_kernel, dim3((unsigned)std::min<size_t>(cdiv(P0, (size_t)WAVES), 256 * 32)), dim3(WG), 0, stream(),
                           ch_in.pieces.p, P0, ch_in.fps.p, d_qlen, d_tlen, ext_rows(o), flag.p);
        DBuf<uint32_t> lidx(P0);
        const size_t n_long = select_flagged_indices(flag.p, lidx.p, P0);
        if (n_long && n_long * 10 <= P0) {
            DeferredPieces::Part part;
            part.pieces.alloc(n_long);
            DBuf<uint32_t> nfp(n_long), off(n_long);
            hipLaunchKernelGGL(gather_pieces_kernel, grid1(n_long), dim3(WG), 0, stream(), ch_in.pieces.p, lidx.p, n_long, part.pieces.p, nfp.p);
            exclusive_scan_u32(nfp.p, off.p, n_long);
            const size_t n_fp_long = (size_t)download_one(off.p + (n_long - 1)) + (size_t)download_one(nfp.p + (n_long - 1));
            part.fps.alloc(n_fp_long);
            if (defer->n_fp + n_fp_long >= (1ull << 32)) fail(HLMI_EINVAL, "more than 2^32 fixed points in the set-aside alignment pieces");
            hipLaunchKernelGGL(move_fixed_points_kernel, dim3((unsigned)std::min<size_t>(cdiv(n_long, (size_t)WAVES), 256 * 32)), dim3(WG), 0, stream(),
                               part.pieces.p, n_long, off.p, (uint32_t)defer->n_fp, ch_in.fps.p, part.fps.p);
            part.n_pieces = n_long; part.n_fp = n_fp_long; part.fp_base = defer->n_fp;
            defer->n_pieces += n_long; defer->n_fp += n_fp_long;
            defer->parts.push_back(std::move(part));
            hipLaunchKernelGGL(class_flag_kernel, grid1(P0), dim3(WG), 0, stream(), flag.p, P0, (uint8_t)0, nflag.p);
            DBuf<uint32_t> kidx(P0);
            const size_t n_keep = select_flagged_indices(nflag.p, kidx.p, P0);
            kept.pieces.alloc(n_keep ? n_keep : 1);
            if (n_keep) hipLaunchKernelGGL(gather_pieces_kernel, grid1(n_keep), dim3(WG), 0, stream(), ch_in.pieces.p, kidx.p, n_keep, kept.pieces.p,
                                           (uint32_t *)nullptr);
            HIP_CHECK(hipGetLastError());
            sync();
            kept.n_pieces = n_keep; kept.n_fp = ch_in.n_fp - n_fp_long;
            stat_add("align_pieces_deferred", (double)n_long);
            if (!n_keep) return;
            chp = &kept;
        }
    }
    const ChainOut &ch = *chp;
    const FixPt *fps_base = ch_in.fps.p;
    const size_t P = ch.n_pieces;
    size_t span_tasks = 64u << 20;
    if (const char *e = hook("HLMI_ALIGN_SPAN_TASKS")) span_tasks = (size_t)std::max(64, atoi(e));
    const size_t NT = ch.n_fp + P;
    if (NT <= span_tasks) {
        AlignOut ao;
        align_span(in, o, d_qlen, d_tlen, PieceSpan{{ch.pieces.p}, P, ch.n_fp, {fps_base}}, ao);
        if (ao.n_rows) outs.push_back(std::move(ao));
        return;
    }
    DBuf<uint32_t> tcnt(P), toff(P);
    hipLaunchKernelGGL(piece_task_count_kernel, dim3((unsigned)cdiv(P, (size_t)256)), dim3(256), 0, stream(), ch.pieces.p, P, tcnt.p);
    exclusive_scan_u32(tcnt.p, toff.p, P);
    const size_t n_spans = (NT + span_tasks - 1) / span_tasks;
    size_t p0 = 0, t0 = 0;
    for (size_t k = 1; k <= n_spans && p0 < P; ++k) {
        size_t p1 = P, t1 = NT;
        if (k < n_spans) {
            const size_t want = NT / n_spans * k;
            size_t lo = p0 + 1, hi = P;
            while (lo < hi) {
                const size_t mid = (lo + hi) / 2;
                if ((size_t)download_one(toff.p + mid) < want) lo = mid + 1; else hi = mid;
            }
            p1 = lo;
            t1 = p1 < P ? (size_t)download_one(toff.p + p1) : NT;
        }
        AlignOut ao;
        align_span(in, o, d_qlen, d_tlen, PieceSpan{{ch.pieces.p + p0}, p1 - p0, (t1 - t0) - (p1 - p0), {fps_base}}, ao);
        if (ao.n_rows) outs.push_back(std::move(ao));
        p0 = p1; t0 = t1;
    }
    stat_add("align_spans", (double)n_spans);
}
}
```

### hylight_amd/csrc/runtime.cpp

```cpp
#include <mutex>

#include "common.h"
#include <sched.h>

#include <iterator>

namespace hlmi {

namespace {
thread_local std::string g_last_error;
bool g_ready = false;
int g_device = 0;
int g_threads = 0;
std::map<std::string, double> g_stats;
std::mutex g_mu;
std::mutex g_stat_mu;

struct KRec { std::string name; hipEvent_t a, b; hipStream_t s; };
struct Lane {
    hipStream_t stream = nullptr, side = nullptr;
    std::vector<KRec> krecs;
    void *pinned = nullptr;
};
Lane g_lanes[MAX_LANES];
thread_local int t_lane = 0;
inline Lane &lane() { return g_lanes[t_lane]; }
}

void set_last_error(const std::string &m) { g_last_error = m; }
const std::string &last_error() { return g_last_error; }

int host_threads() {
    if (g_threads <= 0) {
        cpu_set_t set;
        int n = 8;
        if (sched_getaffinity(0, sizeof set, &set) == 0) n = CPU_COUNT(&set);
        g_threads = std::max(1, std::min(n, 16));
    }
    return g_threads;
}

void *pinned_scratch() {
    void *&p = lane().pinned;
    if (!p) HIP_CHECK(hipHostMalloc(&p, PINNED_SCRATCH_BYTES, hipHostMallocDefault));
    return p;
}

void init_device(int device, int threads) {
    std::lock_guard<std::mutex> lk(g_mu);
    int n = 0;
    hipError_t e = hipGetDeviceCount(&n);
    if (e != hipSuccess || n <= 0)
        fail(HLMI_ENODEV, "no HIP device available (%s); libhylight_mi has no CPU fallback",
             e != hipSuccess ? hipGetErrorString(e) : "device count is 0");
    if (device >= n) fail(HLMI_EINVAL, "device %d out of range (have %d)", device, n);
    if (device >= 0) HIP_CHECK(hipSetDevice(device));
    HIP_CHECK(hipGetDevice(&g_device));
    if (!g_lanes[0].stream) HIP_CHECK(hipStreamCreateWithFlags(&g_lanes[0].stream, hipStreamNonBlocking));
    if (threads > 0) g_threads = threads;
    g_ready = true;
}

void shutdown_device() {
    std::lock_guard<std::mutex> lk(g_mu);
    dev_pool_trim();
    for (Lane &l : g_lanes) {
        for (hipStream_t *st : {&l.side, &l.stream}) {
            if (!*st) continue;
            (void)hipStreamSynchronize(*st);
            (void)hipStreamDestroy(*st);
            *st = nullptr;
        }
    }
    g_ready = false;
}

void require_device() {
    if (!g_ready) init_device(-1, 0);
}

hipStream_t stream() { return lane().stream; }
hipStream_t side_stream_if_created() { return lane().side; }
hipStream_t side_stream() {
    hipStream_t &g_side = lane().side;
    if (!g_side) {
        int least = 0, greatest = 0;
        if (hipDeviceGetStreamPriorityRange(&least, &greatest) != hipSuccess) { (void)hipGetLastError(); greatest = 0; }
        HIP_CHECK(hipStreamCreateWithPriority(&g_side, hipStreamNonBlocking, greatest));
    }
    return g_side;
}

static void lane_drain() {
    Lane &l = lane();
    if (l.stream) (void)hipStreamSynchronize(l.stream);
    if (l.side) (void)hipStreamSynchronize(l.side);
}

KTimer::KTimer(const char *name, hipStream_t on) {
    KRec r;
    r.name = name;
    r.s = on ? on : lane().stream;
    HIP_CHECK(hipEventCreate(&r.a));
    HIP_CHECK(hipEventCreate(&r.b));
    HIP_CHECK(hipEventRecord(r.a, r.s));
    slot = lane().krecs.size();
    lane().krecs.push_back(r);
}
KTimer::~KTimer() { (void)hipEventRecord(lane().krecs[slot].b, lane().krecs[slot].s); }

void ktimer_flush() {
    auto &krecs = lane().krecs;
    if (krecs.empty()) return;
    lane_drain();
    std::lock_guard<std::mutex> lk(g_stat_mu);
    for (auto &r : krecs) {
        float ms = 0;
        if (hipEventElapsedTime(&ms, r.a, r.b) == hipSuccess) {
            g_stats["kernel_ms." + r.name] += ms;
            g_stats["kernel_launches." + r.name] += 1;
        }
        (void)hipEventDestroy(r.a);
        (void)hipEventDestroy(r.b);
    }
    krecs.clear();
}

size_t ktimer_mark() { return lane().krecs.size(); }
void ktimer_rollback(size_t mark) {
    auto &krecs = lane().krecs;
    if (mark >= krecs.size()) return;
    lane_drain();
    for (size_t i = mark; i < krecs.size(); ++i) { (void)hipEventDestroy(krecs[i].a); (void)hipEventDestroy(krecs[i].b); }
    krecs.resize(mark);
}

void ktimer_discard() {
    auto &krecs = lane().krecs;
    if (krecs.empty()) return;
    lane_drain();
    for (auto &r : krecs) { (void)hipEventDestroy(r.a); (void)hipEventDestroy(r.b); }
    krecs.clear();
}

int lane_count() {
    int n = 2;
    if (const char *e = hook("HLMI_LANES")) n = atoi(e);
    return std::max(1, std::min(n, MAX_LANES));
}
LaneScope::LaneScope(int id) : prev(t_lane) {
    if (id < 0 || id >= MAX_LANES) fail(HLMI_EINVAL, "lane %d out of range", id);
    t_lane = id;
    HIP_CHECK(hipSetDevice(g_device));
    if (!lane().stream) HIP_CHECK(hipStreamCreateWithFlags(&lane().stream, hipStreamNonBlocking));
}
LaneScope::~LaneScope() {
    lane_drain();
    try { ktimer_flush(); } catch (...) {}
    t_lane = prev;
}

namespace {
const char *const HOOK_NAMES[] = {
    "HLMI_ALIGN_SPAN_TASKS",
    "HLMI_ANCHOR_BATCH_M",
    "HLMI_ANCHOR_PAIRS",
    "HLMI_ANCHOR_SPLIT",
    "HLMI_ASM_STAGE_CAP",
    "HLMI_ASM_WAVE",
    "HLMI_CHAIN_DP16_CHECK",
    "HLMI_CHAIN_NO_DP16",
    "HLMI_CHAIN_NO_SMALL",
    "HLMI_SEED_GROUP", "HLMI_TEXT_GPU", "HLMI_TEXT_HOST", "HLMI_GRAPH_WINDOW_MB", "HLMI_LANES", "HLMI_SET_ASIDE_CUTS", "HLMI_SEED_NO_GUESS",
    "HLMI_CHAIN_PROF",
    "HLMI_CHAIN_UNPACKED",
    "HLMI_GROUP_HIST",
    "HLMI_HOST_TIMERS",
    "HLMI_LONG_SIDE_STREAM",
    "HLMI_NARROW_LONG_UNPACKED",
    "HLMI_NARROW_UNPACKED",
    "HLMI_NO_EXT_CERT",
    "HLMI_NO_GAP1_CERT",
    "HLMI_NO_GAP2_CERT",
    "HLMI_NO_ONE_PIECE_CERT",
    "HLMI_NO_RANK_WORD",
    "HLMI_NO_SHIFT_CERT",
    "HLMI_NO_STUB",
    "HLMI_NO_SUFFIX_TRIM",
    "HLMI_QCAP_MIN",
    "HLMI_RUN_BUF_CAP",
    "HLMI_SKETCH_PART_MBASES",
    "HLMI_SNP_SORT",
    "HLMI_STUB_FULL_ROWS",
    "HLMI_SUBRUN_MAX_MANCHORS",
    "HLMI_SUBRUN_MAX_OUT_MB",
    "HLMI_SUBRUN_MBASES"};
std::unordered_map<std::string, std::string> g_hooks;
}
void hooks_refresh() {
    g_hooks.clear();
    for (const char *n : HOOK_NAMES)
        if (const char *v = getenv(n)) g_hooks[n] = v;
}
const char *hook(const char *name) {
    bool known = false;
    for (const char *n : HOOK_NAMES) known = known || strcmp(n, name) == 0;
    if (!known) fail(HLMI_EINVAL, "hook %s is not in the table of runtime.cpp", name);
    auto it = g_hooks.find(name);
    return it == g_hooks.end() ? nullptr : it->second.c_str();
}

namespace {
struct CachedBlock { void *p; int lane; };
std::multimap<size_t, CachedBlock> g_free_blocks;
std::mutex g_pool_mu;
std::unordered_map<void *, size_t> g_block_size;
size_t g_pooled_bytes = 0;
size_t g_owned_bytes = 0;
size_t g_peak_in_use = 0;
constexpr size_t POOL_CAP = 160ull << 30;
constexpr size_t GRAN = 2ull << 20;
}

static size_t size_class(size_t bytes) {
    size_t want = (bytes + GRAN - 1) / GRAN * GRAN;
    if (want > (64ull << 20)) {
        size_t p2 = 1;
        while ((p2 << 1) <= want) p2 <<= 1;
        const size_t step = p2 >> 3;
        want = (want + step - 1) / step * step;
    }
    return want;
}

static void pool_trim_locked() {
    (void)hipDeviceSynchronize();
    for (auto &kv : g_free_blocks) {
        (void)hipFree(kv.second.p);
        g_owned_bytes -= kv.first;
        g_block_size.erase(kv.second.p);
    }
    g_free_blocks.clear();
    g_pooled_bytes = 0;
}

void *dev_alloc(size_t bytes) {
    const size_t want = size_class(bytes);
    std::lock_guard<std::mutex> lk(g_pool_mu);
    auto it = g_free_blocks.lower_bound(want);
    {
        int looked = 0;
        for (auto own = it; own != g_free_blocks.end() && own->first <= want + want / 2 && looked < 16; ++own, ++looked)
            if (own->second.lane == t_lane) { it = own; break; }
    }
    if (it != g_free_blocks.end() && it->first <= want + want / 2) {
        void *p = it->second.p;
        const int from = it->second.lane;
        if (from != t_lane && g_lanes[from].stream && lane().stream) {
            hipEvent_t ev;
            HIP_CHECK(hipEventCreateWithFlags(&ev, hipEventDisableTiming));
            HIP_CHECK(hipEventRecord(ev, g_lanes[from].stream));
            HIP_CHECK(hipStreamWaitEvent(lane().stream, ev, 0));
            if (lane().side) HIP_CHECK(hipStreamWaitEvent(lane().side, ev, 0));
            HIP_CHECK(hipEventDestroy(ev));
        }
        g_pooled_bytes -= it->first;
        g_free_blocks.erase(it);
        g_peak_in_use = std::max(g_peak_in_use, g_owned_bytes - g_pooled_bytes);
        return p;
    }
    if (!g_free_blocks.empty()) {
        size_t free_b = 0, total_b = 0;
        if (hipMemGetInfo(&free_b, &total_b) == hipSuccess) {
            bool drained = false;
            while (free_b < want + (1ull << 30) && !g_free_blocks.empty()) {
                if (!drained) { (void)hipDeviceSynchronize(); drained = true; }
                auto big = std::prev(g_free_blocks.end());
                (void)hipFree(big->second.p);
                g_block_size.erase(big->second.p);
                g_pooled_bytes -= big->first;
                g_owned_bytes -= big->first;
                free_b += big->first;
                g_free_blocks.erase(big);
            }
        } else (void)hipGetLastError();
    }
    void *p = nullptr;
    hipError_t e = hipMalloc(&p, want);
    if (e != hipSuccess) {
        (void)hipGetLastError();
        pool_trim_locked();
        e = hipMalloc(&p, want);
        if (e != hipSuccess) (void)hipGetLastError();
    }
    if (e != hipSuccess) fail(HLMI_ENOMEM, "hipMalloc of %zu bytes failed: %s", want, hipGetErrorString(e));
    g_block_size[p] = want;
    g_owned_bytes += want;
    g_peak_in_use = std::max(g_peak_in_use, g_owned_bytes - g_pooled_bytes);
    return p;
}

size_t dev_peak_bytes(bool reset) {
    std::lock_guard<std::mutex> lk(g_pool_mu);
    const size_t v = g_peak_in_use;
    if (reset) g_peak_in_use = g_owned_bytes - g_pooled_bytes;
    return v;
}

size_t dev_available_bytes() {
    size_t free_b = 0, total_b = 0;
    if (hipMemGetInfo(&free_b, &total_b) != hipSuccess) { (void)hipGetLastError(); return 0; }
    std::lock_guard<std::mutex> lk(g_pool_mu);
    return free_b + g_pooled_bytes;
}

void dev_free(void *p) {
    std::lock_guard<std::mutex> lk(g_pool_mu);
    auto it = g_block_size.find(p);
    if (it == g_block_size.end()) { (void)hipFree(p); return; }
    if (g_pooled_bytes + it->second > POOL_CAP) {
        (void)hipFree(p);
        g_owned_bytes -= it->second;
        g_block_size.erase(it);
        return;
    }
    g_free_blocks.emplace(it->second, CachedBlock{p, t_lane});
    g_pooled_bytes += it->second;
}

void dev_pool_trim() {
    std::lock_guard<std::mutex> lk(g_pool_mu);
    pool_trim_locked();
}

static double wall_s() {
    timespec ts;
    clock_gettime(CLOCK_MONOTONIC, &ts);
    return (double)ts.tv_sec + 1e-9 * (double)ts.tv_nsec;
}
static bool host_timers_on() {
    const bool on = hook("HLMI_HOST_TIMERS") != nullptr;
    return on;
}
HostTimer::HostTimer(const char *n) : name(n), t0(0) {
    if (!host_timers_on()) return;
    if (lane().stream) (void)hipStreamSynchronize(lane().stream);
    t0 = wall_s();
}
HostTimer::~HostTimer() {
    if (!host_timers_on()) return;
    if (lane().stream) (void)hipStreamSynchronize(lane().stream);
    stat_add(std::string("host_s.") + name, wall_s() - t0);
}

void stat_reset() { std::lock_guard<std::mutex> lk(g_stat_mu); g_stats.clear(); }
void stat_set(const std::string &k, double v) { std::lock_guard<std::mutex> lk(g_stat_mu); g_stats[k] = v; }
void stat_add(const std::string &k, double v) { std::lock_guard<std::mutex> lk(g_stat_mu); g_stats[k] += v; }
std::map<std::string, double> &stats() { return g_stats; }

}
```

### hylight_amd/csrc/sketch.hip

```cpp
#include "ava.h"
#include "dev_prims.h"

namespace hlmi {

namespace {
constexpr int WG = 256;
inline dim3 grid1(size_t n) { return dim3(cdiv(n ? n : 1, WG)); }

__global__ void encode_kernel(uint8_t *b, size_t n) {
    size_t i = blockIdx.x * (size_t)blockDim.x + threadIdx.x;
    if (i >= n) return;
    uint8_t c = b[i], v = 4;
    switch (c) {
        case 'A': case 'a': v = 0; break;
        case 'C': case 'c': v = 1; break;
        case 'G': case 'g': v = 2; break;
        case 'T': case 't': case 'U': case 'u': v = 3; break;
        default: v = 4;
    }
    b[i] = v;
}

__global__ void mark_read_last_kernel(const uint64_t *off, size_t n_reads, uint8_t *flag) {
    size_t r = blockIdx.x * (size_t)blockDim.x + threadIdx.x;
    if (r >= n_reads) return;
    if (off[r + 1] > off[r]) flag[off[r + 1] - 1] = 1;
}

__global__ void slot_flag_kernel(const uint8_t *codes, size_t n, int hpc, uint8_t *flag) {
    size_t i = blockIdx.x * (size_t)blockDim.x + threadIdx.x;
    if (i >= n) return;
    uint8_t c = codes[i];
    bool end = flag[i] || c > 3 || !hpc || (i + 1 < n && codes[i + 1] != c);
    flag[i] = end ? 1 : 0;
}

__device__ __forceinline__ size_t lower_bound_u32(const uint32_t *a, size_t n, uint64_t v) {
    size_t lo = 0, hi = n;
    while (lo < hi) {
        size_t m = (lo + hi) >> 1;
        if ((uint64_t)a[m] < v) lo = m + 1; else hi = m;
    }
    return lo;
}

__global__ void read_slot0_kernel(const uint32_t *slot_pos, size_t ns, const uint64_t *off, size_t n_reads,
                                  uint32_t *rslot0) {
    size_t r = blockIdx.x * (size_t)blockDim.x + threadIdx.x;
    if (r > n_reads) return;
    rslot0[r] = (uint32_t)lower_bound_u32(slot_pos, ns, off[r]);
}

__global__ void slot_read_kernel(const uint32_t *rslot0, size_t n_reads, size_t ns, uint32_t *slot_rid) {
    size_t s = blockIdx.x * (size_t)blockDim.x + threadIdx.x;
    if (s >= ns) return;
    size_t lo = 0, hi = n_reads;
    while (hi - lo > 1) {
        size_t m = (lo + hi) >> 1;
        if (rslot0[m] <= s) lo = m; else hi = m;
    }
    slot_rid[s] = (uint32_t)lo;
}

__device__ __forceinline__ uint64_t hash64(uint64_t key, uint64_t mask) {
    key = (~key + (key << 21)) & mask;
    key = key ^ key >> 24;
    key = ((key + (key << 3)) + (key << 8)) & mask;
    key = key ^ key >> 14;
    key = ((key + (key << 2)) + (key << 4)) & mask;
    key = key ^ key >> 28;
    key = (key + (key << 31)) & mask;
    return key;
}

__global__ __launch_bounds__(WG) void kmer_kernel(const uint8_t *codes, const uint64_t *off, const uint32_t *slot_pos,
                                                   const uint32_t *slot_rid, const uint32_t *rslot0, size_t ns, int k, int w, int hpc,
                                                   uint64_t *sx, uint32_t *spz, uint8_t *sl) {
    __shared__ uint8_t s_c[WG + 96];
    const int need = w + k - 1;
    const size_t j0 = blockIdx.x * (size_t)WG;
    for (int i = threadIdx.x; i < WG + need - 1; i += WG) {
        const long long si = (long long)j0 - (need - 1) + i;
        s_c[i] = si >= 0 && (size_t)si < ns ? codes[slot_pos[si]] : (uint8_t)4;
    }
    __syncthreads();
    size_t s = j0 + threadIdx.x;
    if (s >= ns) return;
    const uint32_t r = slot_rid[s];
    const size_t s0 = rslot0[r];
    int l = 0;
    uint64_t fwd = 0, rev = 0;
    const uint64_t mask = (1ULL << 2 * k) - 1;
    const int shift = 2 * (k - 1);
    while (l < need && s >= s0 + (size_t)l) {
        uint8_t c = s_c[threadIdx.x + need - 1 - l];
        if (c > 3) break;
        if (l < k) {
            fwd |= (uint64_t)c << (2 * l);
            rev |= (uint64_t)(3 ^ c) << (shift - 2 * l);
        }
        ++l;
    }
    uint64_t x = ~0ull;
    uint32_t pz = 0;
    if (l >= k) {
        const uint64_t pos = slot_pos[s];
        int64_t prev_end = (s >= s0 + (size_t)k) ? (int64_t)slot_pos[s - k] : (int64_t)off[r] - 1;
        int64_t span = hpc ? (int64_t)pos - prev_end : k;
        fwd &= mask;
        if (span < 256 && fwd != rev) {
            int z = fwd < rev ? 0 : 1;
            x = hash64(z ? rev : fwd, mask) << 8 | (uint64_t)span;
            pz = (uint32_t)(pos - off[r]) << 1 | (uint32_t)z;
        }
    }
    sx[s] = x;
    spz[s] = pz;
    sl[s] = (uint8_t)l;
}

__global__ __launch_bounds__(WG) void pick_kernel(const uint64_t *sx, const uint8_t *sl, const uint32_t *slot_rid,
                                                   const uint32_t *rslot0, size_t ns, int k, int w, uint8_t *pick) {
    __shared__ uint64_t s_x[WG + 128];
    __shared__ uint64_t s_wm[WG + 64];
    const size_t j0 = blockIdx.x * (size_t)WG;
    const long long lo = (long long)j0 - (w - 1);
    for (int i = threadIdx.x; i < WG + 2 * (w - 1); i += WG) {
        const long long s = lo + i;
        s_x[i] = s >= 0 && (size_t)s < ns ? sx[s] : ~0ull;
    }
    __syncthreads();
    for (int i = threadIdx.x; i < WG + w - 1; i += WG) {
        const size_t s = j0 + (size_t)i;
        uint64_t mn = ~0ull;
        if (s < ns && (int)sl[s] >= w + k - 1)
            for (int t = 0; t < w; ++t) { const uint64_t v = s_x[i + w - 1 - t]; mn = v < mn ? v : mn; }
        else mn = 0;
        s_wm[i] = mn;
    }
    __syncthreads();
    const size_t j = j0 + threadIdx.x;
    if (j >= ns) return;
    const uint64_t xj = s_x[threadIdx.x + w - 1];
    bool sel = false;
    if (xj != ~0ull) {
        const size_t send = rslot0[slot_rid[j] + 1];
        for (int d = 0; d < w && j + (size_t)d < send && !sel; ++d) {
            const uint64_t m = s_wm[threadIdx.x + d];
            sel = m == xj && (int)sl[j + (size_t)d] >= w + k - 1;
        }
    }
    pick[j] = sel ? 1 : 0;
}

__global__ void emit_mz_kernel(const uint32_t *midx, size_t n, const uint64_t *sx, const uint32_t *spz,
                               const uint32_t *slot_rid, uint32_t rid_base, Mz *out) {
    size_t i = blockIdx.x * (size_t)blockDim.x + threadIdx.x;
    if (i >= n) return;
    uint32_t s = midx[i];
    out[i].x = sx[s];
    out[i].y = (uint64_t)(rid_base + slot_rid[s]) << 32 | spz[s];
}

__global__ void read_count_kernel(const uint32_t *midx, size_t n_mz, const uint32_t *rslot0, size_t n_reads,
                                  uint32_t *counts) {
    size_t r = blockIdx.x * (size_t)blockDim.x + threadIdx.x;
    if (r >= n_reads) return;
    counts[r] = (uint32_t)(lower_bound_u32(midx, n_mz, rslot0[r + 1]) - lower_bound_u32(midx, n_mz, rslot0[r]));
}
}

static void finish_upload(const char *bases, const std::vector<uint64_t> &off, DevReads &out) {
    out.n = off.size() - 1;
    out.total = off.back();
    out.h_off = off;
    out.alloc_codes();
    if (out.total) {
        HIP_CHECK(hipMemcpyAsync(out.codes(), bases, out.total, hipMemcpyHostToDevice, stream()));
        for (uint64_t o = 0; o < out.total; o += 1ull << 30) {
            const uint64_t len = std::min<uint64_t>(1ull << 30, out.total - o);
            hipLaunchKernelGGL(encode_kernel, grid1(len), dim3(WG), 0, stream(), out.codes() + o, len);
        }
        HIP_CHECK(hipGetLastError());
    }
    out.off.upload(off);
    sync();
}

void upload_reads(const SeqSet &s, size_t lo, size_t hi, DevReads &out) {
    std::vector<uint64_t> off(hi - lo + 1);
    for (size_t i = lo; i <= hi; ++i) off[i - lo] = s.off[i] - s.off[lo];
    finish_upload(s.bases.data() + s.off[lo], off, out);
}

void upload_reads(const SeqSet &s, const std::vector<uint32_t> &ids, DevReads &out) {
    std::vector<uint64_t> off(ids.size() + 1, 0);
    std::string bases;
    for (size_t i = 0; i < ids.size(); ++i) {
        bases.append(s.bases, s.off[ids[i]], s.off[ids[i] + 1] - s.off[ids[i]]);
        off[i + 1] = bases.size();
    }
    finish_upload(bases.data(), off, out);
}

__global__ void copy_reads_kernel(const uint8_t *src, const uint64_t *src_off, const uint32_t *ids, const uint64_t *dst_off,
                                  uint8_t *dst) {
    const uint32_t r = blockIdx.x;
    const uint64_t s0 = src_off[ids[r]], d0 = dst_off[r], len = dst_off[r + 1] - d0;
    for (uint64_t i = threadIdx.x; i < len; i += blockDim.x) dst[d0 + i] = src[s0 + i];
}

void subset_reads_device(const DevReads &all, const std::vector<uint32_t> &ids, DevReads &out) {
    std::vector<uint64_t> off(ids.size() + 1, 0);
    for (size_t i = 0; i < ids.size(); ++i) off[i + 1] = off[i] + (all.h_off[ids[i] + 1] - all.h_off[ids[i]]);
    out.n = ids.size();
    out.total = off.back();
    out.h_off = off;
    out.alloc_codes();
    out.off.upload(off);
    if (!ids.empty()) {
        DBuf<uint32_t> d_ids;
        d_ids.upload(ids);
        hipLaunchKernelGGL(copy_reads_kernel, dim3((unsigned)ids.size()), dim3(WG), 0, stream(), all.codes(), all.off.p,
                           d_ids.p, out.off.p, out.codes());
        HIP_CHECK(hipGetLastError());
        sync();
    }
}

static int64_t sketch_core(const DevReads &r, int k, int w, int hpc, uint32_t rid_base, Mz *d_out, int64_t cap,
                           uint32_t *d_counts, DBuf<Mz> *own_out) {
    if (!(k & 1) || k < 3 || k > 28 || w < 1 || w > 64) fail(HLMI_EINVAL, "sketch needs odd k in [3,28], w in [1,64]");
    const size_t n = r.total;
    if (!r.n) return 0;
    if (n >= (1ull << 32)) fail(HLMI_EINVAL, "sketch of %zu bases in one piece (the kernels index bases with 32 bits: the job sketches in parts)", n);
    if (!n) {
        HIP_CHECK(hipMemsetAsync(d_counts, 0, r.n * 4, stream()));
        sync();
        return 0;
    }
    DBuf<uint8_t> flag(n);
    flag.zero();
    hipLaunchKernelGGL(mark_read_last_kernel, grid1(r.n), dim3(WG), 0, stream(), r.off.p, r.n, flag.p);
    hipLaunchKernelGGL(slot_flag_kernel, grid1(n), dim3(WG), 0, stream(), r.codes(), n, hpc, flag.p);
    DBuf<uint32_t> slot_pos(n);
    const size_t ns = select_flagged_indices(flag.p, slot_pos.p, n);
    flag.release();
    KTimer kt_all("sketch_kmer_window");
    DBuf<uint32_t> rslot0(r.n + 1), slot_rid(ns);
    hipLaunchKernelGGL(read_slot0_kernel, grid1(r.n + 1), dim3(WG), 0, stream(), slot_pos.p, ns, r.off.p, r.n, rslot0.p);
    hipLaunchKernelGGL(slot_read_kernel, grid1(ns), dim3(WG), 0, stream(), rslot0.p, r.n, ns, slot_rid.p);
    DBuf<uint64_t> sx(ns);
    DBuf<uint32_t> spz(ns);
    DBuf<uint8_t> sl(ns), pick(ns);
    hipLaunchKernelGGL(kmer_kernel, grid1(ns), dim3(WG), 0, stream(), r.codes(), r.off.p, slot_pos.p, slot_rid.p,
                       rslot0.p, ns, k, w, hpc, sx.p, spz.p, sl.p);
    hipLaunchKernelGGL(pick_kernel, grid1(ns), dim3(WG), 0, stream(), sx.p, sl.p, slot_rid.p, rslot0.p, ns, k, w, pick.p);
    HIP_CHECK(hipGetLastError());
    DBuf<uint32_t> midx(ns);
    const size_t nm = select_flagged_indices(pick.p, midx.p, ns);
    if (own_out) {
        own_out->alloc(nm ? nm : 1);
        d_out = own_out->p;
    } else if ((int64_t)nm > cap) {
        fail(HLMI_EINVAL, "sketch buffer too small: need %zu entries, have %lld", nm, (long long)cap);
    }
    hipLaunchKernelGGL(emit_mz_kernel, grid1(nm), dim3(WG), 0, stream(), midx.p, nm, sx.p, spz.p, slot_rid.p, rid_base,
                       d_out);
    hipLaunchKernelGGL(read_count_kernel, grid1(r.n), dim3(WG), 0, stream(), midx.p, nm, rslot0.p, r.n, d_counts);
    HIP_CHECK(hipGetLastError());
    sync();
    stat_add("sketch_bases", (double)n);
    stat_add("sketch_minimizers", (double)nm);
    return (int64_t)nm;
}

void sketch_device(const DevReads &r, int k, int w, int hpc, uint32_t rid_base, DevSketch &out) {
    out.counts.alloc(r.n ? r.n : 1);
    out.n = (size_t)sketch_core(r, k, w, hpc, rid_base, nullptr, 0, out.counts.p, &out.mz);
}

int64_t sketch_device_into(const DevReads &r, int k, int w, int hpc, uint32_t rid_base, Mz *d_out, int64_t cap,
                           uint32_t *d_counts) {
    return sketch_core(r, k, w, hpc, rid_base, d_out, cap, d_counts, nullptr);
}

}
```

### hylight_amd/csrc/stage.cpp

```cpp
#include "stage.h"

#include <memory>
#include <string_view>
#include <thread>

#include <algorithm>
#include <chrono>

#include "ava.h"
#include "filter_stage.h"
#include "paf_io.h"
#include "row_text.h"

namespace hlmi {

struct Job::Impl {
    SeqSet Q, T_own;
    SeqSet &T;
    explicit Impl(bool same) : T(same ? Q : T_own) {}
    size_t n_bases_q = 0;
    bool long_mode = true;
    hlmi_ava_opts opts{};
    std::vector<std::pair<uint32_t, uint32_t>> chunks;
    std::vector<uint32_t> rank_q, rank_t;
    std::vector<std::string> name_of_rank;
    DevReads dQ, dT_own;
    DevReads *dT = nullptr;
    DBuf<uint32_t> d_rank_q;
    DevSketch own;
    const Mz *d_qmz = nullptr;
    std::vector<uint64_t> qmz_off;
    double est_anchors_per_base = 0, est_out_per_base = 0;
    std::vector<std::unique_ptr<std::string>> text_cache;
    DevNames d_names;
};

static double now_s() {
    return std::chrono::duration<double>(std::chrono::steady_clock::now().time_since_epoch()).count();
}

Job::Job(const char *reads_fa, const char *ref_fa, int nsplit, bool long_mode)
    : impl_(new Impl(std::string(reads_fa) == ref_fa)) {
    Impl &m = *impl_;
    m.long_mode = long_mode;
    m.opts = long_mode ? ava_opts_long() : ava_opts_short();
    m.opts.stub_oh = hook("HLMI_NO_STUB") ? -1 : FilterCfg().v4_min_o;
    read_seqs(reads_fa, m.Q);
    const bool same = std::string(reads_fa) == ref_fa;
    if (!same) read_seqs(ref_fa, m.T);
    m.n_bases_q = m.Q.bases.size();
    name_ranks(m.T.names, m.Q.names, m.rank_t, m.rank_q, m.name_of_rank);
    const uint64_t nu = m.T.n_lines;
    const uint64_t per = (nu / (8ull * (uint64_t)nsplit) + 1) * 8;
    for (size_t r = 0; r < m.T.size();) {
        const uint64_t c = m.T.first_line[r] / per;
        size_t e = r;
        while (e < m.T.size() && m.T.first_line[e] / per == c) ++e;
        const uint64_t end_line = e < m.T.size() ? m.T.first_line[e] : std::max<uint64_t>(nu, m.T.first_line[e - 1] + 1);
        if ((end_line - 1) / per != c)
            fail(HLMI_EINVAL, "record %s straddles an --nsplit chunk boundary", m.T.names[e - 1].c_str());
        m.chunks.emplace_back((uint32_t)r, (uint32_t)e);
        r = e;
    }
    upload_reads(m.Q, 0, m.Q.size(), m.dQ);
    if (same) m.dT = &m.dQ;
    else { upload_reads(m.T, 0, m.T.size(), m.dT_own); m.dT = &m.dT_own; }
    std::string().swap(m.Q.bases);
    std::string().swap(m.T.bases);
    m.d_rank_q.upload(m.rank_q);
    if (m.rank_q.empty()) m.d_rank_q.alloc(1);
}

Job::~Job() = default;
size_t Job::num_queries() const { return impl_->Q.size(); }
size_t Job::num_chunks() const { return impl_->chunks.size(); }

int64_t Job::sketch_bound(int64_t lo, int64_t hi) const {
    const Impl &m = *impl_;
    if (lo < 0 || hi < lo || (size_t)hi > m.Q.size()) fail(HLMI_EINVAL, "sketch range out of bounds");
    return (int64_t)(m.Q.off[hi] - m.Q.off[lo]);
}

int64_t Job::sketch_range(int64_t lo, int64_t hi, void *dev_mz, int64_t cap, void *dev_counts) {
    Impl &m = *impl_;
    if (lo < 0 || hi < lo || (size_t)hi > m.Q.size()) fail(HLMI_EINVAL, "sketch range out of bounds");
    if (lo == hi) return 0;
    uint64_t part_bases = 3ull << 30;
    if (const char *e = hook("HLMI_SKETCH_PART_MBASES")) part_bases = (uint64_t)std::max(1, atoi(e)) << 20;
    const uint64_t bases = m.Q.off[hi] - m.Q.off[lo];
    if (lo == 0 && (size_t)hi == m.Q.size() && bases <= part_bases)
        return sketch_device_into(m.dQ, m.opts.k, m.opts.w, m.opts.hpc, 0, (Mz *)dev_mz, cap, (uint32_t *)dev_counts);
    int64_t total = 0;
    for (int64_t a = lo; a < hi;) {
        int64_t b = a + 1;
        while (b < hi && m.Q.off[b + 1] - m.Q.off[a] <= part_bases) ++b;
        DevReads part;
        std::vector<uint32_t> ids((size_t)(b - a));
        for (size_t i = 0; i < ids.size(); ++i) ids[i] = (uint32_t)(a + (int64_t)i);
        subset_reads_device(m.dQ, ids, part);
        total += sketch_device_into(part, m.opts.k, m.opts.w, m.opts.hpc, (uint32_t)a, (Mz *)dev_mz + total, cap - total,
                                    (uint32_t *)dev_counts + (a - lo));
        a = b;
    }
    return total;
}

void Job::set_query_sketch(const void *dev_mz, int64_t n, const void *dev_counts) {
    Impl &m = *impl_;
    std::vector<uint32_t> cnt(m.Q.size());
    if (!cnt.empty()) {
        HIP_CHECK(hipMemcpyAsync(cnt.data(), dev_counts, cnt.size() * 4, hipMemcpyDeviceToHost, stream()));
        sync();
    }
    m.qmz_off.assign(m.Q.size() + 1, 0);
    for (size_t i = 0; i < cnt.size(); ++i) m.qmz_off[i + 1] = m.qmz_off[i] + cnt[i];
    if ((int64_t)m.qmz_off.back() != n) fail(HLMI_EINVAL, "query sketch has %lld entries but counts sum to %llu", (long long)n,
                                             (unsigned long long)m.qmz_off.back());
    m.d_qmz = (const Mz *)dev_mz;
}

void Job::sketch_all_queries() {
    Impl &m = *impl_;
    uint64_t part_bases = 3ull << 30;
    if (const char *e = hook("HLMI_SKETCH_PART_MBASES")) part_bases = (uint64_t)std::max(1, atoi(e)) << 20;
    if (m.Q.off.back() <= part_bases) {
        sketch_device(m.dQ, m.opts.k, m.opts.w, m.opts.hpc, 0, m.own);
    } else {
        const size_t nq = m.Q.size();
        std::vector<DevSketch> parts;
        std::vector<size_t> first;
        size_t total = 0;
        for (size_t a = 0; a < nq;) {
            size_t b = a + 1;
            while (b < nq && m.Q.off[b + 1] - m.Q.off[a] <= part_bases) ++b;
            DevReads part;
            std::vector<uint32_t> ids(b - a);
            for (size_t i = 0; i < ids.size(); ++i) ids[i] = (uint32_t)(a + i);
            subset_reads_device(m.dQ, ids, part);
            parts.emplace_back();
            sketch_device(part, m.opts.k, m.opts.w, m.opts.hpc, (uint32_t)a, parts.back());
            first.push_back(a);
            total += parts.back().n;
            a = b;
        }
        m.own.mz.alloc(total ? total : 1);
        m.own.counts.alloc(nq ? nq : 1);
        size_t at = 0;
        for (size_t p = 0; p < parts.size(); ++p) {
            const size_t n_reads = (p + 1 < parts.size() ? first[p + 1] : nq) - first[p];
            if (parts[p].n) HIP_CHECK(hipMemcpyAsync(m.own.mz.p + at, parts[p].mz.p, parts[p].n * sizeof(Mz), hipMemcpyDeviceToDevice, stream()));
            HIP_CHECK(hipMemcpyAsync(m.own.counts.p + first[p], parts[p].counts.p, n_reads * 4, hipMemcpyDeviceToDevice, stream()));
            at += parts[p].n;
        }
        sync();
        m.own.n = total;
    }
    set_query_sketch(m.own.mz.p, (int64_t)m.own.n, m.own.counts.p);
}

void Job::run(int rank, int world, int len_over, int mc, double iden, const char *out_paf) {
    Impl &m = *impl_;
    if (!m.d_qmz && m.Q.size()) fail(HLMI_ESTATE, "hlmi_job_run before a query sketch was installed");
    ktimer_discard();
    stat_reset();
    (void)dev_peak_bytes(true);
    const double t0 = now_s();
    struct ExitStamp { double t0; ~ExitStamp() { stat_set("t_with_cleanup_s", now_s() - t0); } } exit_stamp{t0};
    std::vector<uint32_t> my_chunks;
    for (size_t c = 0; c < m.chunks.size(); ++c)
        if ((int)(c % (size_t)world) == rank) my_chunks.push_back((uint32_t)c);
    constexpr double SUBRUN_ANCHORS = 2.0e10;
    double SUBRUN_OUT_BYTES = 52e9;
    bool lanes_fit = false;
    if (const size_t avail = dev_available_bytes()) {
        const double plan = 12.0 * (m.qmz_off.empty() ? 0.0 : (double)m.qmz_off.back());
        SUBRUN_OUT_BYTES = std::min(52e9, std::max(8e9, ((double)avail - plan - 60e9) / (1.5 * 1.5)));
        lanes_fit = (double)avail - plan >= 285e9;
        stat_set("lanes_fit", lanes_fit ? 1 : 0);
    }
    stat_set("subrun_out_budget_gb", SUBRUN_OUT_BYTES / 1e9);
    constexpr uint64_t SUBRUN_MAX_TARGETS = 1u << 20, SUBRUN_MAX_BASES = 3ull << 30;
    double subrun_anchors_max = 4.0e10, subrun_out_max = 1.5 * SUBRUN_OUT_BYTES;
    if (const char *e = hook("HLMI_SUBRUN_MAX_MANCHORS")) subrun_anchors_max = 1e6 * std::max(1e-3, atof(e));
    if (const char *e = hook("HLMI_SUBRUN_MAX_OUT_MB")) subrun_out_max = 1e6 * std::max(1e-3, atof(e));
    const double subrun_anchors = std::min(SUBRUN_ANCHORS, subrun_anchors_max / 2), subrun_out = std::min(SUBRUN_OUT_BYTES, subrun_out_max / 1.5);
    uint64_t budget_bases = 128ull << 20;
    if (const char *e = hook("HLMI_SUBRUN_MBASES")) budget_bases = (uint64_t)std::max(1, atoi(e)) << 20;
    const bool fixed_budget = hook("HLMI_SUBRUN_MBASES") != nullptr;
    if (!fixed_budget && m.est_anchors_per_base > 0) {
        const double by_anchors = subrun_anchors / m.est_anchors_per_base;
        const double by_bytes = m.est_out_per_base > 0 ? subrun_out / m.est_out_per_base : by_anchors;
        budget_bases = std::min<uint64_t>(SUBRUN_MAX_BASES, std::max<uint64_t>(4ull << 20, (uint64_t)(0.9 * std::min(by_anchors, by_bytes))));
    }
    std::vector<std::string_view> lines;
    std::vector<uint32_t> line_keys;
    std::vector<std::unique_ptr<std::string>> text;
    std::vector<uint32_t> tids;
    double t_ava = 0, t_flt = 0, t_fmt = 0, t_dl = 0;
    size_t n_v4 = 0, n_ev = 0, n_pairs = 0, n_subruns = 0;
    uint64_t done_bases = 0;
    double done_anchors = 0, done_out_bytes = 0;
    for (size_t ci = 0; ci < my_chunks.size() && m.Q.size();) {
        std::vector<uint32_t> sub_tids, chunk_of_t;
        uint32_t n_my = 0;
        uint64_t sub_bases = 0, sub_real_bases = 0;
        const double n_names = (double)std::max<size_t>(1, m.name_of_rank.size());
        while (ci < my_chunks.size()) {
            const auto &ch = m.chunks[my_chunks[ci]];
            const uint64_t cb_real = m.T.off[ch.second] - m.T.off[ch.first];
            uint64_t cb = cb_real;
            if (m.opts.pair_once) {
                double w = 0;
                for (uint32_t t = ch.first; t < ch.second; ++t) w += (double)m.T.len(t) * 2.0 * ((double)m.rank_t[t] + 0.5) / n_names;
                cb = (uint64_t)w + 1;
            }
            if (n_my && (sub_bases + cb > budget_bases || sub_real_bases + cb_real > SUBRUN_MAX_BASES ||
                         sub_tids.size() + (ch.second - ch.first) > SUBRUN_MAX_TARGETS)) break;
            for (uint32_t t = ch.first; t < ch.second; ++t) { sub_tids.push_back(t); chunk_of_t.push_back(n_my); }
            sub_bases += cb;
            sub_real_bases += cb_real;
            ++n_my; ++ci;
        }
        if (sub_tids.empty()) continue;
        const double ts0 = now_s();
        DevReads dT_sub;
        const bool all_in_order = sub_tids.size() == m.T.size();
        if (!all_in_order) subset_reads_device(*m.dT, sub_tids, dT_sub);
        DevReads &dT = all_in_order ? *m.dT : dT_sub;
        std::vector<uint32_t> rt(sub_tids.size());
        for (size_t i = 0; i < sub_tids.size(); ++i) rt[i] = m.rank_t[sub_tids[i]];
        DBuf<uint32_t> d_rt, d_ct;
        d_rt.upload(rt);
        d_ct.upload(chunk_of_t);
        AvaInput in;
        in.T = &dT; in.Q = &m.dQ; in.d_rank_t = d_rt.p; in.d_rank_q = m.d_rank_q.p; in.d_chunk_of_t = d_ct.p;
        in.n_chunks = n_my; in.d_qmz = m.d_qmz; in.qmz_off = m.qmz_off;
        in.n_ranks = m.name_of_rank.size();
        if (m.dT == &m.dQ) in.t_query = sub_tids;
        in.max_anchors = (uint64_t)subrun_anchors_max;
        in.max_out_bytes = (uint64_t)subrun_out_max;
        in.max_lanes = lanes_fit ? 0 : 1;
        AvaRows rows;
        const double a0 = stats()["anchors"];
        const std::map<std::string, double> stats_before = stats();
        const size_t timers_before = ktimer_mark();
        ava_device(in, m.opts, rows);
        if (rows.refused_anchors) {
            budget_bases = std::max<uint64_t>(1, (uint64_t)(rows.refused_shrink * (double)sub_bases));
            ci -= n_my;
            stats() = stats_before;
            ktimer_rollback(timers_before);
            stat_add("subruns_refused", 1);
            continue;
        }
        tids.insert(tids.end(), sub_tids.begin(), sub_tids.end());
        ++n_subruns;
        done_bases += sub_bases;
        done_anchors += stats()["anchors"] - a0;
        done_out_bytes += (double)ava_out_bytes(rows.n_rows, rows.n_ops);
        if (!fixed_budget && done_anchors > 0) {
            const double by_anchors = subrun_anchors * (double)done_bases / done_anchors;
            const double by_bytes = done_out_bytes > 0 ? subrun_out * (double)done_bases / done_out_bytes : by_anchors;
            budget_bases = std::min<uint64_t>(SUBRUN_MAX_BASES, std::max<uint64_t>(subrun_anchors < SUBRUN_ANCHORS || subrun_out < SUBRUN_OUT_BYTES ? 1 : 4ull << 20, (uint64_t)std::min(by_anchors, by_bytes)));
        }
        const double t1 = now_s();
        t_ava += t1 - ts0;
        FilterCfg cfg;
        cfg.len_over = len_over; cfg.mc = mc; cfg.long_mode = m.long_mode;
        cfg.chunk_id_bound = n_my;
        cfg.reference_order = false;
        const std::vector<uint64_t> chunk_ops = ops_per_chunk(rows.recs.p, rows.n_rows, n_my);
        FilterOut fo;
        double t_fmt_sub = 0;
        for (uint32_t c0 = 0; c0 < n_my;) {
            uint32_t c1 = c0;
            uint64_t ops = 0;
            while (c1 < n_my && (c1 == c0 || ops + chunk_ops[c1] <= (1ull << 30))) ops += chunk_ops[c1++];
            const uint64_t r0 = rows.chunk_row_start[c0], r1 = rows.chunk_row_start[c1];
            std::vector<uint64_t> crs(rows.chunk_row_start.begin() + c0, rows.chunk_row_start.begin() + c1 + 1);
            for (auto &v : crs) v -= r0;
            filter_stage_device(rows.recs.p + r0, (size_t)(r1 - r0), rows.ops_base, crs, cfg, fo);
            n_v4 += fo.n_after_v4; n_ev += fo.n_events; n_pairs += fo.n_pairs;
            const double tf = now_s();
            const bool text_on_gpu = !hook("HLMI_TEXT_HOST") && (fo.rows.size() >= 65536 || hook("HLMI_TEXT_GPU"));
            if (text_on_gpu) {
                if (!m.d_names.n) m.d_names.upload(m.name_of_rank);
                RowText rt;
                format_rows_device(rows.recs.p + r0, fo.rows, fo.x_digit_sum, m.d_names, iden, rt);
                t_dl += now_s() - tf;
                std::unique_ptr<std::string> extra(new std::string());
                std::vector<std::pair<size_t, std::pair<size_t, size_t>>> extra_at;
                for (size_t i = 0; i < fo.rows.size(); ++i)
                    if (rt.len[i] == ROW_TEXT_TO_HOST) {
                        const std::vector<PafRec> one = download_rows(rows.recs.p + r0, std::vector<uint32_t>(1, fo.rows[i]));
                        std::string tmp;
                        uint32_t k = 0;
                        if (format_scored_row(one[0], m.name_of_rank[one[0].qid], m.name_of_rank[one[0].tid], fo.x_digit_sum[i], iden, tmp, &k)) {
                            extra_at.push_back({i, {extra->size(), tmp.size()}});
                            extra->append(tmp);
                            rt.key[i] = k;
                        }
                    }
                stat_add("rows_text_on_gpu", (double)fo.rows.size());
                stat_add("rows_text_left_to_host", (double)extra_at.size());
                text.emplace_back(new std::string(std::move(rt.text)));
                const std::string &buf = *text.back();
                text.emplace_back(std::move(extra));
                const std::string &ebuf = *text.back();
                size_t e = 0;
                lines.reserve(lines.size() + fo.rows.size());
                line_keys.reserve(line_keys.size() + fo.rows.size());
                for (size_t i = 0; i < fo.rows.size(); ++i) {
                    if (rt.len[i] == ROW_TEXT_TO_HOST) {
                        if (e < extra_at.size() && extra_at[e].first == i) {
                            lines.emplace_back(ebuf.data() + extra_at[e].second.first, extra_at[e].second.second);
                            line_keys.push_back(rt.key[i]);
                            ++e;
                        }
                    } else if (rt.len[i]) { lines.emplace_back(buf.data() + rt.at[i], rt.len[i]); line_keys.push_back(rt.key[i]); }
                }
            } else {
            std::vector<PafRec> kept = download_rows(rows.recs.p + r0, fo.rows);
            t_dl += now_s() - tf;
            {
                const size_t nk = kept.size();
                std::vector<uint32_t> at(nk), len(nk, 0), key(nk);
                const int nt = (int)std::max<size_t>(1, std::min<size_t>((size_t)host_threads(), nk / 2048));
                const size_t first_buf = text.size();
                for (int t = 0; t < nt; ++t) {
                    if (!m.text_cache.empty()) { text.emplace_back(std::move(m.text_cache.back())); m.text_cache.pop_back(); text.back()->clear(); }
                    else text.emplace_back(new std::string());
                }
                auto work = [&](int t) {
                    std::string tmp, &buf = *text[first_buf + (size_t)t];
                    buf.reserve((nk / nt + 1) * 160);
                    for (size_t i = nk * (size_t)t / nt; i < nk * (size_t)(t + 1) / nt; ++i)
                        if (format_scored_row(kept[i], m.name_of_rank[kept[i].qid], m.name_of_rank[kept[i].tid],
                                              fo.x_digit_sum[i], iden, tmp, &key[i])) {
                            at[i] = (uint32_t)buf.size(); len[i] = (uint32_t)tmp.size();
                            buf.append(tmp);
                        }
                };
                std::vector<std::thread> pool;
                for (int t = 1; t < nt; ++t) pool.emplace_back(work, t);
                work(0);
                for (auto &th : pool) th.join();
                lines.reserve(lines.size() + nk);
                line_keys.reserve(line_keys.size() + nk);
                for (int t = 0; t < nt; ++t) {
                    const std::string &buf = *text[first_buf + (size_t)t];
                    for (size_t i = nk * (size_t)t / nt; i < nk * (size_t)(t + 1) / nt; ++i)
                        if (len[i]) { lines.emplace_back(buf.data() + at[i], len[i]); line_keys.push_back(key[i]); }
                }
            }
            }
            t_fmt_sub += now_s() - tf;
            c0 = c1;
        }
        t_fmt += t_fmt_sub;
        t_flt += now_s() - t1 - t_fmt_sub;
    }
    if (done_bases && done_anchors > 0) {
        m.est_anchors_per_base = done_anchors / (double)done_bases;
        m.est_out_per_base = done_out_bytes / (double)done_bases;
    }
    stat_set("subruns", (double)n_subruns);
    stat_set("rows_after_v4", (double)n_v4);
    stat_set("snp_events", (double)n_ev);
    stat_set("pairs", (double)n_pairs);
    stat_set("t_ava_s", t_ava);
    stat_set("t_filter_s", t_flt);
    stat_set("t_rows_to_text_s", t_fmt);
    stat_set("t_rows_download_s", t_dl);
    const double t3 = now_s();
    sort_scored_lines(lines, &line_keys);
    stat_set("t_final_sort_s", now_s() - t3);
    write_lines(out_paf, lines);
    {
        std::sort(text.begin(), text.end(), [](const auto &a, const auto &b) { return a->capacity() > b->capacity(); });
        size_t held = 0;
        for (auto &b : m.text_cache) held += b->capacity();
        for (auto &b : text)
            if (held + b->capacity() <= (2ull << 30) && m.text_cache.size() < 64) { held += b->capacity(); m.text_cache.emplace_back(std::move(b)); }
        lines.clear();
        text.clear();
    }
    stat_set("rows_out", (double)line_keys.size());
    stat_set("t_format_sort_write_s", now_s() - t3);
    ktimer_flush();
    stat_set("t_total_s", now_s() - t0);
    stat_set("hbm_peak_in_use_gb", (double)dev_peak_bytes(false) / 1e9);

    stat_set("bases_q", (double)m.n_bases_q);
    uint64_t bt = 0;
    for (uint32_t t : tids) bt += m.T.len(t);
    stat_set("bases_t", (double)bt);
    stat_set("targets", (double)tids.size());
    stat_set("queries", (double)m.Q.size());
    stat_set("minimizers_q", m.qmz_off.empty() ? 0.0 : (double)m.qmz_off.back());
    stat_set("chunks_run", (double)my_chunks.size());
}

}
```

Before: 3567.

## Compare reads in classify pass using packed 2-bit codes and ambiguity flags

Adds a 2-bit packed copy of each read set plus a per-32-base ambiguity bitmap, built at upload and subset time. The classify kernel's mismatch scan and shift checks then load 32 bases per 64-bit word instead of 8 bases per word whenever no window in the wave touches an ambiguous base, cutting memory traffic and ALU work per base. The cost is an extra pack kernel, extra device memory for the packed copy (accounted for in the lanes-fit budget), duplicated template paths, and a fallback to the byte path whenever any lane in the wave hits an N.

```diff
diff --git a/hylight_amd/csrc/ava.h b/hylight_amd/csrc/ava.h
--- a/hylight_amd/csrc/ava.h
+++ b/hylight_amd/csrc/ava.h
@@ -44,12 +44,20 @@
         HIP_CHECK(hipMemsetAsync(store.p, 4, PAD, stream()));
         HIP_CHECK(hipMemsetAsync(store.p + PAD + total, 4, PAD, stream()));
     }
+    DBuf<uint8_t> packed_store;
+    DBuf<uint32_t> nflag;
+    const uint8_t *packed() const { return packed_store.p + PAD / 4; }
+    void pack();
+    static uint64_t packed_bytes(uint64_t total) {
+        const uint64_t n_gran = (total + 2 * PAD + 31) / 32;
+        return (n_gran + 2) * 8 + ((n_gran + 31) / 32 + 2) * 4;
+    }
     DBuf<uint64_t> off;
     std::vector<uint64_t> h_off;
 };
 void upload_reads(const SeqSet &s, size_t lo, size_t hi, DevReads &out);
 void upload_reads(const SeqSet &s, const std::vector<uint32_t> &ids, DevReads &out);
-void subset_reads_device(const DevReads &all, const std::vector<uint32_t> &ids, DevReads &out);
+void subset_reads_device(const DevReads &all, const std::vector<uint32_t> &ids, DevReads &out, bool pack = true);
 
 struct DevSketch {
     size_t n = 0;
diff --git a/hylight_amd/csrc/ava_align.hip b/hylight_amd/csrc/ava_align.hip
--- a/hylight_amd/csrc/ava_align.hip
+++ b/hylight_amd/csrc/ava_align.hip
@@ -134,6 +134,8 @@
     size_t n_list;
     const uint8_t *qcodes, *tcodes;
     long long q_total, t_total;
+    const uint8_t *qpacked, *tpacked;
+    const uint32_t *qnflag, *tnflag;
     int match, mismatch, go, ge, ambi;
     int go2, ge2;
     int end_bonus;
@@ -210,7 +212,7 @@
 }
 
 
-enum { ST_BASES = 0, ST_BASES_SQUARE, ST_BASES_NARROW, ST_BASES_WIDE, ST_FAST, ST_DP, ST_DP_ROWS, ST_NARROW_SMALL, ST_WIDE_ONE, ST_STUB_EXT, ST_EXT_CERT, ST_EXT_DP_ROW, ST_EXT_DP_K, ST_LONG, ST_BASES_LONG, N_ALIGN_STATS };
+enum { ST_BASES = 0, ST_BASES_SQUARE, ST_BASES_NARROW, ST_BASES_WIDE, ST_FAST, ST_DP, ST_DP_ROWS, ST_NARROW_SMALL, ST_WIDE_ONE, ST_STUB_EXT, ST_EXT_CERT, ST_EXT_DP_ROW, ST_EXT_DP_K, ST_LONG, ST_BASES_LONG, ST_PACKED, N_ALIGN_STATS };
 constexpr int NR_SMALL = 64;
 constexpr uint8_t CLS_LONG = 5;
 constexpr uint8_t CLS_LONG32 = 7;
@@ -246,18 +248,65 @@
     return v;
 }
 
+__device__ __forceinline__ uint64_t load_window32p(const uint8_t *packed, long long a0, bool down, bool comp, int x) {
+    const long long s = down ? a0 - x - 31 : a0 + x;
+    const uint8_t *p = packed + (s >> 2);
+    uint64_t lo;
+    __builtin_memcpy(&lo, p, 8);
+    const int sh = 2 * (int)(s & 3);
+    uint64_t v = lo >> sh | (uint64_t)p[8] << 1 << (63 - sh);
+    if (down) {
+        v = __builtin_bitreverse64(v);
+        v = (v >> 1 & 0x5555555555555555ull) | (v & 0x5555555555555555ull) << 1;
+    }
+    return comp ? ~v : v;
+}
+__device__ __forceinline__ uint32_t ne_bits32(uint64_t q, uint64_t t) {
+    const uint64_t d = q ^ t;
+    auto even = [](uint32_t x) {
+        x = (x | x >> 1) & 0x55555555u;
+        x = (x | x >> 1) & 0x33333333u;
+        x = (x | x >> 2) & 0x0f0f0f0fu;
+        x = (x | x >> 4) & 0x00ff00ffu;
+        return (x | x >> 8) & 0xffffu;
+    };
+    return even((uint32_t)d) | even((uint32_t)(d >> 32)) << 16;
+}
+__device__ __forceinline__ uint32_t squeeze8(uint64_t f) {
+    return (((uint32_t)f * 0x10204080u) >> 28) | (((uint32_t)(f >> 32) * 0x10204080u) >> 28) << 4;
+}
+__device__ __forceinline__ uint32_t ne_bits8(uint64_t q, uint64_t t) {
+    const uint64_t d = q ^ t;
+    return squeeze8((d | d >> 1 | d >> 2) & 0x0101010101010101ull);
+}
+__device__ __forceinline__ uint32_t amb_bits8(uint64_t q, uint64_t t) { return squeeze8((q | t) >> 2 & 0x0101010101010101ull); }
+__device__ __forceinline__ bool range_flagged(const uint32_t *nflag, long long lo, long long hi) {
+    const uint32_t g0 = (uint32_t)((lo + (long long)DevReads::PAD) >> 5), g1 = (uint32_t)((hi + (long long)DevReads::PAD) >> 5);
+    uint32_t any = 0;
+    for (uint32_t w = g0 >> 5; w <= g1 >> 5; ++w) {
+        uint32_t keep = ~0u;
+        if (w == g0 >> 5) keep &= ~0u << (g0 & 31);
+        if (w == g1 >> 5) keep &= ~0u >> (31 - (g1 & 31));
+        any |= nflag[w] & keep;
+    }
+    return any != 0;
+}
+__device__ __forceinline__ bool window_flagged(const uint32_t *nflag, long long a0, bool down, int len) {
+    return down ? range_flagged(nflag, a0 - (len - 1), a0) : range_flagged(nflag, a0, a0 + (len - 1));
+}
+
 template <int PASS>
 __global__ __launch_bounds__(WG) __attribute__((amdgpu_waves_per_eu(PASS == 1 ? 4 : 5))) void classify_kernel(AlignArgs a, uint8_t *cls, unsigned long long *stats) {
     __shared__ unsigned long long s_stat[WAVES][N_ALIGN_STATS];
-    constexpr int CMP_PIECES = PASS == 1 ? 64 * (BLOCK_MAX / 8) : 1;
-    __shared__ uint8_t s_mm[WAVES][CMP_PIECES], s_up[WAVES][CMP_PIECES], s_dn[WAVES][CMP_PIECES];
+    constexpr int CMP_WORDS = PASS == 1 ? 64 * (BLOCK_MAX / 32) : 1;
+    __shared__ uint32_t s_mm[WAVES][CMP_WORDS], s_up[WAVES][CMP_WORDS], s_dn[WAVES][CMP_WORDS];
     __shared__ uint64_t s_qa[WAVES][PASS == 1 ? 64 : 1], s_ta[WAVES][PASS == 1 ? 64 : 1];
     __shared__ uint32_t s_geo[WAVES][PASS == 1 ? 64 : 1], s_amb[WAVES][2];
     const int lane = threadIdx.x & 63;
     const size_t tid = blockIdx.x * (size_t)blockDim.x + threadIdx.x;
     const size_t n_thr = (size_t)gridDim.x * blockDim.x;
     uint32_t chunk_off = 0, chunk_left = 0;
-    uint32_t st[N_ALIGN_STATS] = {0, 0, 0, 0, 0, 0, 0, 0, 0, 0, 0, 0, 0, 0, 0};
+    uint32_t st[N_ALIGN_STATS] = {};
     const size_t n_units = PASS == 1 ? a.n_tasks : (size_t)*a.defer_count;
     const size_t rounds = (n_units + n_thr - 1) / n_thr;
     TaskRef ref_n{0, 0};
@@ -310,82 +359,102 @@
         bool ambig = false, shift_ok = false;
         if constexpr (PASS == 1) {
             const int wv = threadIdx.x >> 6;
-            uint8_t *own = s_mm[wv], *mm = s_mm[wv], *mup = s_up[wv], *mdn = s_dn[wv];
-            const uint32_t nch = try_fast ? (uint32_t)(m + 7) >> 3 : 0u;
+            bool flagged = false;
+            if (try_fast && a.qpacked)
+                flagged = window_flagged(a.qnflag, (long long)tk.qa, (tk.kind & TASK_REV) != 0, m) || window_flagged(a.tnflag, (long long)tk.ta, false, m);
+            const bool use_packed = a.qpacked != nullptr && __ballot(flagged) == 0;
+            uint32_t *mm = s_mm[wv], *mup = s_up[wv], *mdn = s_dn[wv];
+            const uint32_t nch = try_fast ? (uint32_t)(m + 31) >> 5 : 0u;
             const uint32_t incl = wave_prefix_sum_incl_dpp(nch), tot = (uint32_t)__builtin_amdgcn_readlane((int)incl, 63);
             const uint32_t st0 = incl - nch;
-            for (uint32_t c = (uint32_t)lane; c < tot; c += 64) own[c] = 0;
             if (lane < 2) s_amb[wv][lane] = 0;
             s_qa[wv][lane] = tk.qa; s_ta[wv][lane] = tk.ta;
-            s_geo[wv][lane] = st0 | (uint32_t)m << 16 | ((tk.kind & TASK_REV) ? 0x80000000u : 0u);
-            __builtin_amdgcn_s_waitcnt(0xc07f);
-            __builtin_amdgcn_wave_barrier();
-            if (nch) own[st0] = (uint8_t)lane;
-            __builtin_amdgcn_s_waitcnt(0xc07f);
-            __builtin_amdgcn_wave_barrier();
-            int carry = 0;
-            constexpr int CU = 4;
-            for (uint32_t c0 = 0; c0 < tot; c0 += 64 * CU) {
-                int ow[CU], xs[CU], left[CU];
-                bool rv[CU];
-#pragma unroll
-                for (int u = 0; u < CU; ++u) {
-                    const uint32_t c = c0 + 64u * u + (uint32_t)lane;
-                    int o = c < tot ? (int)own[c] : 0;
-                    o = wave_prefix_max_incl_dpp(o);
-                    o = o > carry ? o : carry;
-                    carry = __builtin_amdgcn_readlane(o, 63);
-                    const uint32_t geo = s_geo[wv][o];
-                    ow[u] = o;
-                    xs[u] = (int)(c - (geo & 0xffffu)) * 8;
-                    left[u] = c < tot ? (int)(geo >> 16 & 0x7fffu) - xs[u] : 0;
-                    rv[u] = (geo >> 31) != 0;
-                }
-                uint64_t q8[CU], t8[CU];
-                uint32_t q_end = 0, t_end = 0;
-#pragma unroll
-                for (int u = 0; u < CU; ++u) {
-                    q8[u] = t8[u] = 0;
-                    if (left[u] > 0) {
-                        q8[u] = load_window8p(a.qcodes, (long long)s_qa[wv][ow[u]], rv[u], rv[u], xs[u]);
-                        t8[u] = load_window8p(a.tcodes, (long long)s_ta[wv][ow[u]], false, false, xs[u]);
-                        if (u == CU - 1 && lane == 63 && a.kshift) {
-                            q_end = (uint32_t)load_window8p(a.qcodes, (long long)s_qa[wv][ow[u]], rv[u], rv[u], xs[u] + 8) & 0xffu;
-                            t_end = (uint32_t)load_window8p(a.tcodes, (long long)s_ta[wv][ow[u]], false, false, xs[u] + 8) & 0xffu;
+            auto compare = [&](auto packed_form) {
+                constexpr bool PK = decltype(packed_form)::value;
+                constexpr int PB = PK ? 32 : 8, PW = 32 / PB;
+                constexpr uint32_t FIRST = PK ? 3u : 0xffu;
+                using piece_t = std::conditional_t<PK, uint32_t, uint8_t>;
+                piece_t *own = (piece_t *)mm, *pm = (piece_t *)mm, *pup = (piece_t *)mup, *pdn = (piece_t *)mdn;
+                const uint32_t ptot = tot * PW, pst0 = st0 * PW;
+                auto window = [&](bool query, int o, bool rv, int x) {
+                    if constexpr (PK) return query ? load_window32p(a.qpacked, (long long)s_qa[wv][o], rv, rv, x) : load_window32p(a.tpacked, (long long)s_ta[wv][o], false, false, x);
+                    else return query ? load_window8p(a.qcodes, (long long)s_qa[wv][o], rv, rv, x) : load_window8p(a.tcodes, (long long)s_ta[wv][o], false, false, x);
+                };
+                for (uint32_t c = (uint32_t)lane; c < ptot; c += 64) own[c] = 0;
+                s_geo[wv][lane] = pst0 | (uint32_t)m << 16 | ((tk.kind & TASK_REV) ? 0x80000000u : 0u);
+                __builtin_amdgcn_s_waitcnt(0xc07f);
+                __builtin_amdgcn_wave_barrier();
+                if (nch) own[pst0] = (piece_t)lane;
+                __builtin_amdgcn_s_waitcnt(0xc07f);
+                __builtin_amdgcn_wave_barrier();
+                int carry = 0;
+                constexpr int CU = 4;
+                for (uint32_t c0 = 0; c0 < ptot; c0 += 64 * CU) {
+                    int ow[CU], xs[CU], left[CU];
+                    bool rv[CU];
+#pragma unroll
+                    for (int u = 0; u < CU; ++u) {
+                        const uint32_t c = c0 + 64u * u + (uint32_t)lane;
+                        int o = c < ptot ? (int)own[c] : 0;
+                        o = wave_prefix_max_incl_dpp(o);
+                        o = o > carry ? o : carry;
+                        carry = __builtin_amdgcn_readlane(o, 63);
+                        const uint32_t geo = s_geo[wv][o];
+                        ow[u] = o;
+                        xs[u] = (int)(c - (geo & 0xffffu)) * PB;
+                        left[u] = c < ptot ? (int)(geo >> 16 & 0x7fffu) - xs[u] : 0;
+                        rv[u] = (geo >> 31) != 0;
+                    }
+                    uint64_t qw[CU], tw[CU];
+                    uint32_t q_end = 0, t_end = 0;
+#pragma unroll
+                    for (int u = 0; u < CU; ++u) {
+                        qw[u] = tw[u] = 0;
+                        if (left[u] > 0) {
+                            qw[u] = window(true, ow[u], rv[u], xs[u]);
+                            tw[u] = window(false, ow[u], false, xs[u]);
+                            if (u == CU - 1 && lane == 63 && a.kshift) {
+                                q_end = (uint32_t)window(true, ow[u], rv[u], xs[u] + PB) & FIRST;
+                                t_end = (uint32_t)window(false, ow[u], false, xs[u] + PB) & FIRST;
+                            }
                         }
                     }
-                }
-                int nq[CU], nt[CU];
-                if (a.kshift) {
+                    int nq[CU], nt[CU];
+                    if (a.kshift) {
+#pragma unroll
+                        for (int u = 0; u < CU; ++u) {
+                            const int q_after = u + 1 < CU ? __builtin_amdgcn_readlane((int)((uint32_t)qw[u + 1 < CU ? u + 1 : u] & FIRST), 0) : (int)q_end;
+                            const int t_after = u + 1 < CU ? __builtin_amdgcn_readlane((int)((uint32_t)tw[u + 1 < CU ? u + 1 : u] & FIRST), 0) : (int)t_end;
+                            nq[u] = wave_shl1((int)((uint32_t)qw[u] & FIRST), q_after);
+                            nt[u] = wave_shl1((int)((uint32_t)tw[u] & FIRST), t_after);
+                        }
+                    }
 #pragma unroll
                     for (int u = 0; u < CU; ++u) {
-                        const int q_after = u + 1 < CU ? __builtin_amdgcn_readlane((int)((uint32_t)q8[u + 1 < CU ? u + 1 : u] & 0xffu), 0) : (int)q_end;
-                        const int t_after = u + 1 < CU ? __builtin_amdgcn_readlane((int)((uint32_t)t8[u + 1 < CU ? u + 1 : u] & 0xffu), 0) : (int)t_end;
-                        nq[u] = wave_shl1((int)((uint32_t)q8[u] & 0xffu), q_after);
-                        nt[u] = wave_shl1((int)((uint32_t)t8[u] & 0xffu), t_after);
+                        if (left[u] <= 0) continue;
+                        const uint32_t c = c0 + 64u * u + (uint32_t)lane;
+                        if constexpr (PK) {
+                            pm[c] = ne_bits32(qw[u], tw[u]) & (left[u] >= 32 ? ~0u : (1u << left[u]) - 1u);
+                            if (a.kshift) {
+                                const uint64_t q9 = qw[u] >> 2 | (uint64_t)(uint32_t)nq[u] << 62, t9 = tw[u] >> 2 | (uint64_t)(uint32_t)nt[u] << 62;
+                                pup[c] = ne_bits32(q9, tw[u]);
+                                pdn[c] = ne_bits32(qw[u], t9);
+                            }
+                        } else {
+                            const uint64_t keep = left[u] >= 8 ? ~0ull : (1ull << (8 * left[u])) - 1ull;
+                            if ((qw[u] | tw[u]) & keep & 0x0404040404040404ull) atomicOr(&s_amb[wv][ow[u] >> 5], 1u << (ow[u] & 31));
+                            pm[c] = (uint8_t)ne_bits8(qw[u] & keep, tw[u] & keep);
+                            if (a.kshift) {
+                                const uint64_t q9 = qw[u] >> 8 | (uint64_t)(uint32_t)nq[u] << 56, t9 = tw[u] >> 8 | (uint64_t)(uint32_t)nt[u] << 56;
+                                pup[c] = (uint8_t)ne_bits8(q9, tw[u]);
+                                pdn[c] = (uint8_t)ne_bits8(qw[u], t9);
+                            }
+                        }
                     }
                 }
-#pragma unroll
-                for (int u = 0; u < CU; ++u) {
-                    if (left[u] <= 0) continue;
-                    const uint64_t keep = left[u] >= 8 ? ~0ull : (1ull << (8 * left[u])) - 1ull;
-                    uint64_t d = (q8[u] ^ t8[u]) & keep;
-                    if ((q8[u] | t8[u]) & keep & 0x0404040404040404ull) atomicOr(&s_amb[wv][ow[u] >> 5], 1u << (ow[u] & 31));
-                    d = (d | d >> 1 | d >> 2) & 0x0101010101010101ull;
-                    auto squeeze = [](uint64_t f) {
-                        return (uint8_t)((((uint32_t)f * 0x10204080u) >> 28) | (((uint32_t)(f >> 32) * 0x10204080u) >> 28) << 4);
-                    };
-                    mm[c0 + 64u * u + (uint32_t)lane] = squeeze(d);
-                    if (a.kshift) {
-                        const uint64_t q9 = q8[u] >> 8 | (uint64_t)(uint32_t)nq[u] << 56, t9 = t8[u] >> 8 | (uint64_t)(uint32_t)nt[u] << 56;
-                        uint64_t du = q9 ^ t8[u], dd = q8[u] ^ t9;
-                        du = (du | du >> 1 | du >> 2) & 0x0101010101010101ull;
-                        dd = (dd | dd >> 1 | dd >> 2) & 0x0101010101010101ull;
-                        mup[c0 + 64u * u + (uint32_t)lane] = squeeze(du);
-                        mdn[c0 + 64u * u + (uint32_t)lane] = squeeze(dd);
-                    }
-                }
-            }
+            };
+            if (use_packed) { compare(std::true_type{}); if (try_fast) ++st[ST_PACKED]; }
+            else compare(std::false_type{});
             __builtin_amdgcn_s_waitcnt(0xc07f);
             __builtin_amdgcn_wave_barrier();
             if (try_fast) {
@@ -395,7 +464,7 @@
                     while (bits) {
                         const int y = __ffs((int)bits) - 1;
                         bits &= bits - 1;
-                        if (k < 3) mpos[k] = (int)(8 * j) + y;
+                        if (k < 3) mpos[k] = (int)(32 * j) + y;
                         ++k;
                     }
                 }
@@ -403,10 +472,10 @@
             if (try_fast && !ambig && a.kshift && k == a.kmax + 1) {
                 const int p1 = mpos[0], pk = mpos[k - 1];
                 uint32_t any_up = 0, any_dn = 0;
-                for (int j = p1 >> 3; j <= (pk - 1) >> 3; ++j) {
-                    uint32_t keepb = 0xffu;
-                    if (j == p1 >> 3) keepb &= 0xffu << (p1 & 7);
-                    if (j == (pk - 1) >> 3) keepb &= 0xffu >> (7 - ((pk - 1) & 7));
+                for (int j = p1 >> 5; j <= (pk - 1) >> 5; ++j) {
+                    uint32_t keepb = ~0u;
+                    if (j == p1 >> 5) keepb &= ~0u << (p1 & 31);
+                    if (j == (pk - 1) >> 5) keepb &= ~0u >> (31 - ((pk - 1) & 31));
                     any_up |= mup[st0 + (uint32_t)j] & keepb;
                     any_dn |= mdn[st0 + (uint32_t)j] & keepb;
                 }
@@ -415,7 +484,7 @@
             if (try_fast && k > 0 && !ambig) {
                 for (int j = (int)nch - 1; j >= 0; --j) {
                     const uint32_t bits = mm[st0 + (uint32_t)j];
-                    if (bits) { last_x = 8 * j + 31 - __clz((int)bits); break; }
+                    if (bits) { last_x = 32 * j + 31 - __clz((int)bits); break; }
                 }
             }
             __builtin_amdgcn_wave_barrier();
@@ -427,6 +496,18 @@
         int fast_score = a.match * (m - k) - a.mismatch * k;
         uint32_t ext_flag = 0;
         int ext_take = -1;
+        auto pairs = [&](auto packed_form, bool q_down, bool t_down, int xq, int xt, uint32_t &ne, uint32_t &amb) {
+            const bool rev = (tk.kind & TASK_REV) != 0;
+            if constexpr (decltype(packed_form)::value) {
+                ne = ne_bits32(load_window32p(a.qpacked, (long long)tk.qa, q_down, rev, xq), load_window32p(a.tpacked, (long long)tk.ta, t_down, false, xt));
+                amb = 0;
+            } else {
+                const uint64_t q8 = load_window8p(a.qcodes, (long long)tk.qa, q_down, rev, xq), t8 = load_window8p(a.tcodes, (long long)tk.ta, t_down, false, xt);
+                ne = ne_bits8(q8, t8);
+                amb = amb_bits8(q8, t8);
+            }
+        };
+        auto low_bits = [](int n, int w) { return n >= w ? ~0u >> (32 - w) : (1u << n) - 1u; };
         if (PASS == 2 && live && c != 0 && (tk.kind & 3) != 0 && a.kmax >= 0) {
             const bool rev = (tk.kind & TASK_REV) != 0, left = (tk.kind & 3) == 1;
             const int L = m < n ? m : n;
@@ -443,31 +524,30 @@
             const int k_want = bonus_row ? (L == end_row ? a.kext_bonus : 0) : a.kext_plain;
             int x1 = -1, x2 = -1;
             auto more = [&]() { return same || (!amb_ext && (k_ext <= allow || k_ext <= k_want)); };
-            auto take8 = [&](int x, uint64_t q8, uint64_t t8) {
-                const int rest = L - x;
-                const uint64_t keep = rest >= 8 ? ~0ull : (1ull << (8 * rest)) - 1ull;
-                uint64_t d = (q8 ^ t8) & keep;
-                amb_ext |= ((q8 | t8) & keep & 0x0404040404040404ull) != 0;
-                d = (d | d >> 1 | d >> 2) & 0x0101010101010101ull;
-                if (d && x2 < 0) {
-                    const int y1 = (__ffsll((long long)d) - 1) >> 3;
-                    if (x1 < 0) { x1 = x + y1; const uint64_t d2 = d & (d - 1); if (d2) x2 = x + ((__ffsll((long long)d2) - 1) >> 3); }
-                    else x2 = x + y1;
-                }
-                k_ext += __popcll(d);
-                same = same && d == 0 && !amb_ext;
+            auto scan = [&](auto packed_form) {
+                constexpr int W = decltype(packed_form)::value ? 32 : 8;
+                auto take = [&](int x, uint32_t ne, uint32_t amb) {
+                    const uint32_t keep = low_bits(L - x, W);
+                    ne &= keep;
+                    amb_ext |= (amb & keep) != 0;
+                    if (ne && x2 < 0) {
+                        const int y1 = __ffs((int)ne) - 1;
+                        if (x1 < 0) { x1 = x + y1; const uint32_t d2 = ne & (ne - 1); if (d2) x2 = x + __ffs((int)d2) - 1; }
+                        else x2 = x + y1;
+                    }
+                    k_ext += __popc(ne);
+                    same = same && ne == 0 && !amb_ext;
+                };
+                for (int x = 0; x < L && more(); x += 2 * W) {
+                    uint32_t ne0, amb0, ne1 = 0, amb1 = 0;
+                    pairs(packed_form, left != rev, left, x, x, ne0, amb0);
+                    if (x + W < L) pairs(packed_form, left != rev, left, x + W, x + W, ne1, amb1);
+                    take(x, ne0, amb0);
+                    if (x + W < L && more()) take(x + W, ne1, amb1);
+                }
             };
-            for (int x = 0; x < L && more(); x += 16) {
-                const uint64_t q8 = load_window8p(a.qcodes, (long long)tk.qa, left != rev, rev, x);
-                const uint64_t t8 = load_window8p(a.tcodes, (long long)tk.ta, left, false, x);
-                uint64_t q8b = 0, t8b = 0;
-                if (x + 8 < L) {
-                    q8b = load_window8p(a.qcodes, (long long)tk.qa, left != rev, rev, x + 8);
-                    t8b = load_window8p(a.tcodes, (long long)tk.ta, left, false, x + 8);
-                }
-                take8(x, q8, t8);
-                if (x + 8 < L && more()) take8(x + 8, q8b, t8b);
-            }
+            if (a.qpacked && !window_flagged(a.qnflag, (long long)tk.qa, left != rev, L) && !window_flagged(a.tnflag, (long long)tk.ta, left, L)) { scan(std::true_type{}); ++st[ST_PACKED]; }
+            else scan(std::false_type{});
             if (!same && !amb_ext && k_ext <= allow) { tk.kind |= TASK_ONE; ++st[ST_WIDE_ONE]; }
             if (same) {
                 runs[nr++] = (uint32_t)L << 4 | OP_EQ;
@@ -511,38 +591,42 @@
             int found_a = 0, found_b = 0, a1 = mn, a2 = mn, a3 = mn, b1 = -1, b2 = -1, b3 = -1;
             bool amb = false;
             const int sq = m > n ? m - n : 0, st_ = n > m ? n - m : 0;
-            for (int x = 0; x < mn && (found_a < want || found_b < want); x += 8) {
-                const bool da = found_a < want, db = found_b < want;
-                const int e0 = mn - 8 - x;
-                uint64_t q8 = 0, t8 = 0, q8e = 0, t8e = 0;
-                if (da) { q8 = load_window8p(a.qcodes, (long long)tk.qa, rev, rev, x); t8 = load_window8p(a.tcodes, (long long)tk.ta, false, false, x); }
-                if (db) { q8e = load_window8p(a.qcodes, (long long)tk.qa, rev, rev, e0 + sq); t8e = load_window8p(a.tcodes, (long long)tk.ta, false, false, e0 + st_); }
-                const int left = mn - x;
-                if (da) {
-                    const uint64_t keep = left >= 8 ? ~0ull : (1ull << (8 * left)) - 1ull;
-                    amb |= ((q8 | t8) & keep & 0x0404040404040404ull) != 0;
-                    uint64_t d = (q8 ^ t8) & keep;
-                    d = (d | d >> 1 | d >> 2) & 0x0101010101010101ull;
-                    while (d && found_a < want) {
-                        const int y = (__ffsll((long long)d) - 1) >> 3;
-                        d &= d - 1;
-                        if (found_a == 0) a1 = x + y; else if (found_a == 1) a2 = x + y; else a3 = x + y;
-                        ++found_a;
+            auto scan = [&](auto packed_form) {
+                constexpr int W = decltype(packed_form)::value ? 32 : 8;
+                for (int x = 0; x < mn && (found_a < want || found_b < want); x += W) {
+                    const bool da = found_a < want, db = found_b < want;
+                    const int e0 = mn - W - x;
+                    uint32_t ne_a = 0, amb_a = 0, ne_b = 0, amb_b = 0;
+                    if (da) pairs(packed_form, rev, false, x, x, ne_a, amb_a);
+                    if (db) pairs(packed_form, rev, false, e0 + sq, e0 + st_, ne_b, amb_b);
+                    const int left = mn - x;
+                    if (da) {
+                        const uint32_t keep = low_bits(left, W);
+                        amb |= (amb_a & keep) != 0;
+                        uint32_t d = ne_a & keep;
+                        while (d && found_a < want) {
+                            const int y = __ffs((int)d) - 1;
+                            d &= d - 1;
+                            if (found_a == 0) a1 = x + y; else if (found_a == 1) a2 = x + y; else a3 = x + y;
+                            ++found_a;
+                        }
                     }
-                }
-                if (db) {
-                    const uint64_t keep = left >= 8 ? ~0ull : ~0ull << (8 * (8 - left));
-                    amb |= ((q8e | t8e) & keep & 0x0404040404040404ull) != 0;
-                    uint64_t d = (q8e ^ t8e) & keep;
-                    d = (d | d >> 1 | d >> 2) & 0x0101010101010101ull;
-                    while (d && found_b < want) {
-                        const int z = 7 - (__clzll((long long)d) >> 3);
-                        d &= ~(0xffull << (8 * z));
-                        if (found_b == 0) b1 = e0 + z; else if (found_b == 1) b2 = e0 + z; else b3 = e0 + z;
-                        ++found_b;
+                    if (db) {
+                        const uint32_t keep = left >= W ? ~0u : low_bits(W, W) & ~low_bits(W - left, W);
+                        amb |= (amb_b & keep) != 0;
+                        uint32_t d = ne_b & keep;
+                        while (d && found_b < want) {
+                            const int z = 31 - __clz((int)d);
+                            d &= ~(1u << z);
+                            if (found_b == 0) b1 = e0 + z; else if (found_b == 1) b2 = e0 + z; else b3 = e0 + z;
+                            ++found_b;
+                        }
                     }
                 }
-            }
+            };
+            const bool use_packed = a.qpacked && !window_flagged(a.qnflag, (long long)tk.qa, rev, m) && !window_flagged(a.tnflag, (long long)tk.ta, false, n);
+            if (use_packed) { scan(std::true_type{}); ++st[ST_PACKED]; }
+            else scan(std::false_type{});
             int p_star = -1, xpos = -1, xpos2 = -1;
             if (!amb) {
                 if (b1 < a1) p_star = b1 + 1;
@@ -556,23 +640,25 @@
                 else if (a1 < mn && b1 >= 0 && Mab < m2) { ps = Mab + 1; x1 = a1; x2 = b1; }
                 else if (a2 < mn && M2 < a3) { ps = M2 + 1; x1 = a1; x2 = a2; }
                 if (ps >= 0 && a1 < b1) {
-                    auto load_s = [&](int x) { return del ? load_window8p(a.qcodes, (long long)tk.qa, rev, rev, x) : load_window8p(a.tcodes, (long long)tk.ta, false, false, x); };
-                    auto load_l = [&](int x) { return del ? load_window8p(a.tcodes, (long long)tk.ta, false, false, x) : load_window8p(a.qcodes, (long long)tk.qa, rev, rev, x); };
                     bool far_ne = false, near_ne = false, ambx = false;
-                    for (int x = a1; x < b1 && !far_ne; x += 8) {
-                        const uint64_t s8 = load_s(x), l8 = load_l(x + 2);
-                        const int left = b1 - x;
-                        const uint64_t keep = left >= 8 ? ~0ull : (1ull << (8 * left)) - 1ull;
-                        ambx |= ((s8 | l8) & keep & 0x0404040404040404ull) != 0;
-                        far_ne = ((s8 ^ l8) & keep) != 0;
-                    }
-                    for (int x = a1 + 1; x <= b1 && !near_ne; x += 8) {
-                        const uint64_t s8 = load_s(x), l8 = load_l(x - 1);
-                        const int left = b1 + 1 - x;
-                        const uint64_t keep = left >= 8 ? ~0ull : (1ull << (8 * left)) - 1ull;
-                        ambx |= ((s8 | l8) & keep & 0x0404040404040404ull) != 0;
-                        near_ne = ((s8 ^ l8) & keep) != 0;
-                    }
+                    auto shifted = [&](auto packed_form) {
+                        constexpr int W = decltype(packed_form)::value ? 32 : 8;
+                        uint32_t ne, ab;
+                        for (int x = a1; x < b1 && !far_ne; x += W) {
+                            pairs(packed_form, rev, false, del ? x : x + 2, del ? x + 2 : x, ne, ab);
+                            const uint32_t keep = low_bits(b1 - x, W);
+                            ambx |= (ab & keep) != 0;
+                            far_ne = (ne & keep) != 0;
+                        }
+                        for (int x = a1 + 1; x <= b1 && !near_ne; x += W) {
+                            pairs(packed_form, rev, false, del ? x : x - 1, del ? x - 1 : x, ne, ab);
+                            const uint32_t keep = low_bits(b1 + 1 - x, W);
+                            ambx |= (ab & keep) != 0;
+                            near_ne = (ne & keep) != 0;
+                        }
+                    };
+                    if (use_packed) shifted(std::true_type{});
+                    else shifted(std::false_type{});
                     if (far_ne && near_ne && !ambx) { p_star = ps; xpos = x1; xpos2 = x2; }
                 }
             }
@@ -2411,6 +2497,11 @@
         aa.geom = TaskGeom{task_ref.p, pgeom.p, ch.fps.p};
         aa.qcodes = in.Q->codes(); aa.tcodes = in.T->codes();
         aa.q_total = (long long)in.Q->total; aa.t_total = (long long)in.T->total;
+        if (!hook("HLMI_CLASSIFY_BYTES")) {
+            if (!in.Q->packed_store.p || !in.T->packed_store.p) fail(HLMI_ESTATE, "alignment of a read set without its 2-bit copy (DevReads::pack)");
+            aa.qpacked = in.Q->packed(); aa.tpacked = in.T->packed();
+            aa.qnflag = in.Q->nflag.p; aa.tnflag = in.T->nflag.p;
+        }
         aa.end_bonus = o.end_bonus;
         aa.ext_max = ext_rows(o);
         aa.ext_all_long = ext_all_long ? 1 : 0;
@@ -2748,6 +2839,7 @@
     {
         std::vector<unsigned long long> h = astats.download(N_ALIGN_STATS);
         stat_add("align_tasks_fast", (double)h[ST_FAST]);
+        stat_add("align_tasks_packed", (double)h[ST_PACKED]);
         stat_add("align_tasks_dp", (double)h[ST_DP]);
         stat_add("align_dp_rows", (double)h[ST_DP_ROWS]);
         stat_add("align_dp_bases", (double)h[ST_BASES]);
diff --git a/hylight_amd/csrc/runtime.cpp b/hylight_amd/csrc/runtime.cpp
--- a/hylight_amd/csrc/runtime.cpp
+++ b/hylight_amd/csrc/runtime.cpp
@@ -174,6 +174,7 @@
     "HLMI_SEED_GROUP", "HLMI_TEXT_GPU", "HLMI_TEXT_HOST", "HLMI_GRAPH_WINDOW_MB", "HLMI_LANES", "HLMI_SET_ASIDE_CUTS", "HLMI_SEED_NO_GUESS",
     "HLMI_CHAIN_PROF",
     "HLMI_CHAIN_UNPACKED",
+    "HLMI_CLASSIFY_BYTES",
     "HLMI_GROUP_HIST",
     "HLMI_HOST_TIMERS",
     "HLMI_LONG_SIDE_STREAM",
diff --git a/hylight_amd/csrc/sketch.hip b/hylight_amd/csrc/sketch.hip
--- a/hylight_amd/csrc/sketch.hip
+++ b/hylight_amd/csrc/sketch.hip
@@ -170,6 +170,39 @@
 }
 }
 
+__global__ void pack_kernel(const uint8_t *store, uint64_t n_store, uint64_t *packed, uint32_t *nflag, uint64_t n_gran) {
+    const uint64_t g = blockIdx.x * (uint64_t)blockDim.x + threadIdx.x;
+    uint64_t w = 0;
+    bool amb = g >= n_gran;
+    if (!amb) {
+        for (int k = 0; k < 4; ++k) {
+            const uint64_t i = 32 * g + 8 * (uint64_t)k;
+            uint64_t c8 = 0;
+            if (i + 8 <= n_store) __builtin_memcpy(&c8, store + i, 8);
+            else for (int b = 0; b < 8; ++b) c8 |= (uint64_t)(i + b < n_store ? store[i + b] : 4) << (8 * b);
+            amb |= (c8 & 0x0404040404040404ull) != 0;
+            for (int b = 0; b < 8; ++b) w |= (c8 >> (8 * b) & 3ull) << (2 * (8 * k + b));
+        }
+        packed[g] = w;
+    }
+    const uint64_t bits = __ballot(amb);
+    if ((threadIdx.x & 31) == 0 && g < n_gran) nflag[g >> 5] = (uint32_t)(bits >> (threadIdx.x & 32));
+}
+
+void DevReads::pack() {
+    const uint64_t n_store = total + 2 * PAD, n_gran = (n_store + 31) / 32, n_words = (n_gran + 31) / 32;
+    packed_store.alloc((n_gran + 2) * 8);
+    nflag.alloc(n_words + 2);
+    HIP_CHECK(hipMemsetAsync(packed_store.p + n_gran * 8, 0, 16, stream()));
+    HIP_CHECK(hipMemsetAsync(nflag.p + n_words, 0xff, 8, stream()));
+    for (uint64_t g0 = 0; g0 < n_gran; g0 += 1ull << 30) {
+        const uint64_t len = std::min<uint64_t>(1ull << 30, n_gran - g0);
+        hipLaunchKernelGGL(pack_kernel, grid1(len), dim3(WG), 0, stream(), store.p + 32 * g0, n_store - 32 * g0,
+                           (uint64_t *)packed_store.p + g0, nflag.p + g0 / 32, len);
+    }
+    HIP_CHECK(hipGetLastError());
+}
+
 static void finish_upload(const char *bases, const std::vector<uint64_t> &off, DevReads &out) {
     out.n = off.size() - 1;
     out.total = off.back();
@@ -183,6 +216,7 @@
         }
         HIP_CHECK(hipGetLastError());
     }
+    out.pack();
     out.off.upload(off);
     sync();
 }
@@ -210,7 +244,7 @@
     for (uint64_t i = threadIdx.x; i < len; i += blockDim.x) dst[d0 + i] = src[s0 + i];
 }
 
-void subset_reads_device(const DevReads &all, const std::vector<uint32_t> &ids, DevReads &out) {
+void subset_reads_device(const DevReads &all, const std::vector<uint32_t> &ids, DevReads &out, bool pack) {
     std::vector<uint64_t> off(ids.size() + 1, 0);
     for (size_t i = 0; i < ids.size(); ++i) off[i + 1] = off[i] + (all.h_off[ids[i] + 1] - all.h_off[ids[i]]);
     out.n = ids.size();
@@ -224,8 +258,9 @@
         hipLaunchKernelGGL(copy_reads_kernel, dim3((unsigned)ids.size()), dim3(WG), 0, stream(), all.codes(), all.off.p,
                            d_ids.p, out.off.p, out.codes());
         HIP_CHECK(hipGetLastError());
-        sync();
-    }
+    }
+    if (pack) out.pack();
+    sync();
 }
 
 static int64_t sketch_core(const DevReads &r, int k, int w, int hpc, uint32_t rid_base, Mz *d_out, int64_t cap,
diff --git a/hylight_amd/csrc/stage.cpp b/hylight_amd/csrc/stage.cpp
--- a/hylight_amd/csrc/stage.cpp
+++ b/hylight_amd/csrc/stage.cpp
@@ -97,7 +97,7 @@
         DevReads part;
         std::vector<uint32_t> ids((size_t)(b - a));
         for (size_t i = 0; i < ids.size(); ++i) ids[i] = (uint32_t)(a + (int64_t)i);
-        subset_reads_device(m.dQ, ids, part);
+        subset_reads_device(m.dQ, ids, part, false);
         total += sketch_device_into(part, m.opts.k, m.opts.w, m.opts.hpc, (uint32_t)a, (Mz *)dev_mz + total, cap - total,
                                     (uint32_t *)dev_counts + (a - lo));
         a = b;
@@ -136,7 +136,7 @@
             DevReads part;
             std::vector<uint32_t> ids(b - a);
             for (size_t i = 0; i < ids.size(); ++i) ids[i] = (uint32_t)(a + i);
-            subset_reads_device(m.dQ, ids, part);
+            subset_reads_device(m.dQ, ids, part, false);
             parts.emplace_back();
             sketch_device(part, m.opts.k, m.opts.w, m.opts.hpc, (uint32_t)a, parts.back());
             first.push_back(a);
@@ -175,7 +175,8 @@
     if (const size_t avail = dev_available_bytes()) {
         const double plan = 12.0 * (m.qmz_off.empty() ? 0.0 : (double)m.qmz_off.back());
         SUBRUN_OUT_BYTES = std::min(52e9, std::max(8e9, ((double)avail - plan - 60e9) / (1.5 * 1.5)));
-        lanes_fit = (double)avail - plan >= 285e9;
+        const double packed_sub = (double)DevReads::packed_bytes(std::min<uint64_t>(m.T.off.empty() ? 0 : m.T.off.back(), 3ull << 30));
+        lanes_fit = (double)avail - plan - packed_sub >= 285e9;
         stat_set("lanes_fit", lanes_fit ? 1 : 0);
     }
     stat_set("subrun_out_budget_gb", SUBRUN_OUT_BYTES / 1e9);
```

Result: faster. 3671, median of 6 (+2.9%).
